# vganapati/CT_PVAE

Measured on AMD Instinct MI355X. Metric: projections/sec (fwd+adj) 128x128 foam, 20 angles; fraction of HBM roofline, higher is better.
Workload: dtype f32; 1 GPU; batch=50/GPU 128x128 foam, 20 angles, P=184, rotate nearest fwd + tf_compat adj; objects_per_gpu=50, n_pixel=128, angles=20, num_proj_pix=184, parallelism=batch-shard x1, forward_plan=u16 taps, launch=19 replays of a HIP graph of 100 steps + 66 steps launched from Python

## Files before the change

ct_pvae_amd/_lib.py:

```python
import ctypes
import os

_HERE = os.path.dirname(os.path.abspath(__file__))
LIB_PATH = os.path.join(_HERE, "libctpvae_radon.so")

NEAREST, BILINEAR = 0, 1
NOISE = {"gaussian": 0, "poisson": 1}
BWD_TF_COMPAT, BWD_EXACT = 0, 1
SIDDON_STORE = {"raysum": 0, "sirt": 1, "tv_dual": 2, "gaussian": 3, "poisson": 4, "ratio": 5}
EINVAL, EHIP, ENODEV = -1, -2, -3
ABI_VERSION = 3400

_c_int, _c_float, _vp = ctypes.c_int, ctypes.c_float, ctypes.c_void_p
_ip = ctypes.POINTER(ctypes.c_int)

SIGNATURES = {
    "ctpvae_abi_version": (_c_int, []),
    "ctpvae_last_error": (ctypes.c_char_p, []),
    "ctpvae_device_count": (_c_int, []),
    "ctpvae_tune_set": (_c_int, [ctypes.c_char_p, _c_int]),
    "ctpvae_tune_active": (_c_int, []),
    "ctpvae_num_proj_pix": (_c_int, [_c_int, _c_int]),
    "ctpvae_pad_amounts": (_c_int, [_c_int, _c_int, _ip, _ip]),
    "ctpvae_rotate_transforms_f32": (_c_int, [_vp, _c_int, _c_int, _c_int, _vp, _vp, _vp]),
    "ctpvae_rotate_transforms_host_f32": (_c_int, [_vp, _c_int, _c_int, _c_int, _vp, _vp]),
    "ctpvae_rotate_fwd_planned_sel_f32": (_c_int, [_vp, _c_int, _c_int, _c_int, _c_int, _c_int, _c_int, _vp, _vp, _c_int, _vp, _vp]),
    "ctpvae_rotate_fwd_planned_loglik_sel_f32": (_c_int, [_vp, _c_int, _c_int, _c_int, _c_int, _c_int, _c_int, _vp, _vp, _c_int,
                                                          _vp, _vp, _c_int, _vp, _c_float, _vp, _vp, _vp, _vp]),
    "ctpvae_rotate_cplan_supported": (_c_int, [_c_int, _c_int, _c_int, _c_int, _c_int, _c_int]),
    "ctpvae_rotate_cplan_bytes": (ctypes.c_longlong, [_c_int, _c_int, _c_int, _c_int, _c_int]),
    "ctpvae_rotate_cplan_build_f32": (_c_int, [_vp, _c_int, _c_int, _c_int, _c_int, _c_int, _c_int, _c_int, _vp, _vp]),
    "ctpvae_rotate_cplan_overflowed": (_c_int, [_vp, _c_int, _c_int, _c_int, _c_int, _c_int, _vp]),
    "ctpvae_rotate_fwd_compact_f32": (_c_int, [_vp, _c_int, _c_int, _c_int, _c_int, _c_int, _c_int, _vp, _vp, _c_int, _c_int, _vp,
                                               _vp, _c_int, _vp, _c_float, _vp, _vp, _vp, _vp, _vp, _vp]),
    "ctpvae_rotate_fwd_compact_noise_f32": (_c_int, [_vp, _c_int, _c_int, _c_int, _c_int, _c_int, _c_int, _vp, _vp, _c_int, _c_int, _vp,
                                                     _vp, _c_int, _vp, _c_float, _c_int, _vp, _vp, _vp, _vp, _vp, _vp]),
    "ctpvae_loglik_tasks_per_row": (_c_int, [_c_int, _c_int]),
    "ctpvae_loglik_part_floats": (ctypes.c_longlong, [_c_int, _c_int, _c_int, _c_int]),
    "ctpvae_loglik_object_sums_f32": (_c_int, [_vp, _c_int, _c_int, _c_int, _c_int, _vp, _vp]),
    "ctpvae_rotate_bwd_sel_scaled_f32": (_c_int, [_vp, _c_int, _c_int, _c_int, _c_int, _vp, _vp, _c_int, _c_int, _c_int, _c_int,
                                                  _c_int, _vp, ctypes.c_longlong, _vp, _vp]),
    "ctpvae_rotate_bwd4_plan_bytes": (ctypes.c_longlong, [_c_int, _c_int, _c_int, _c_int, _c_int]),
    "ctpvae_rotate_bwd4_plan_build_f32": (_c_int, [_vp, _c_int, _c_int, _c_int, _c_int, _c_int, _c_int, _c_int, _vp, _vp]),
    "ctpvae_rotate_bwd_planned_sel_scaled_f32": (_c_int, [_vp, _c_int, _c_int, _c_int, _c_int, _c_int, _c_int, _vp, _vp, _c_int,
                                                          _c_int, _vp, ctypes.c_longlong, _vp, _vp]),
    "ctpvae_rotate_fwd_f32": (_c_int, [_vp, _c_int, _c_int, _c_int, _c_int, _c_int, _c_int, _c_int, _vp, _c_int,
                                       _c_int, _vp, _vp]),
    "ctpvae_rotate_fwd_f64": (_c_int, [_vp, _c_int, _c_int, _c_int, _c_int, _c_int, _c_int, _c_int, _vp, _c_int,
                                       _c_int, _vp, _vp]),
    "ctpvae_rotate_bwd_f64": (_c_int, [_vp, _c_int, _c_int, _c_int, _c_int, _vp, _c_int, _c_int, _c_int, _c_int,
                                       _c_int, _c_int, _vp, _vp]),
    "ctpvae_rotate_tile_shape": (_c_int, [_c_int, _c_int, _c_int, ctypes.POINTER(ctypes.c_int), ctypes.POINTER(ctypes.c_int)]),
    "ctpvae_rotate_fwd_tiled_workspace_bytes": (ctypes.c_longlong, [_c_int, _c_int, _c_int, _c_int, _c_int, _c_int, _c_int]),
    "ctpvae_rotate_fwd_tiled_f32": (_c_int, [_vp, _c_int, _c_int, _c_int, _c_int, _c_int, _c_int, _c_int, _vp, _c_int, _vp,
                                             _vp, _vp]),
    "ctpvae_rotate_fwd_tiled_interp_f32": (_c_int, [_vp, _c_int, _c_int, _c_int, _c_int, _c_int, _c_int, _c_int, _vp, _c_int, _c_int,
                                                    _vp, _vp, _vp]),
    "ctpvae_rotate_fwd_fast_f32": (_c_int, [_vp, _c_int, _c_int, _c_int, _c_int, _c_int, _c_int, _c_int, _vp, _c_int, _vp, _vp]),
    "ctpvae_rotate_fwd_tiled_fast_f32": (_c_int, [_vp, _c_int, _c_int, _c_int, _c_int, _c_int, _c_int, _c_int, _vp, _c_int, _vp,
                                                  _vp, _vp]),
    "ctpvae_rotate_fwd_tiled_loglik_f32": (_c_int, [_vp, _c_int, _c_int, _c_int, _c_int, _c_int, _c_int, _c_int, _vp, _c_int,
                                                    _vp, _vp, _vp, _vp, _c_float, _vp, _vp, _vp, _vp]),
    "ctpvae_rotate_tplan_bytes": (ctypes.c_longlong, [_c_int, _c_int, _c_int, _c_int, _c_int]),
    "ctpvae_rotate_tplan_build_f32": (_c_int, [_vp, _c_int, _c_int, _c_int, _c_int, _c_int, _c_int, _c_int, _vp, _vp]),
    "ctpvae_rotate_tplan_overflowed": (_c_int, [_vp, _c_int, _c_int, _c_int, _c_int, _c_int, _vp]),
    "ctpvae_rotate_fwd_tiled_compact_f32": (_c_int, [_vp, _c_int, _c_int, _c_int, _c_int, _c_int, _c_int, _c_int, _vp, _c_int, _vp,
                                                     _vp, _vp, _vp, _vp, _c_float, _vp, _vp, _vp, _vp, _vp, _vp]),
    "ctpvae_rotate_bwd_f32": (_c_int, [_vp, _c_int, _c_int, _c_int, _c_int, _vp, _c_int, _c_int, _c_int, _c_int,
                                       _c_int, _c_int, _vp, _vp]),
    "ctpvae_rotate_bwd_scaled_f32": (_c_int, [_vp, _c_int, _c_int, _c_int, _c_int, _vp, _c_int, _c_int, _c_int, _c_int,
                                              _c_int, _c_int, _vp, ctypes.c_longlong, _vp, _vp]),
    "ctpvae_rotate_plan_supported": (_c_int, [_c_int, _c_int, _c_int, _c_int, _c_int, _c_int, _c_int]),
    "ctpvae_rotate_plan_bytes": (ctypes.c_longlong, [_c_int, _c_int, _c_int, _c_int, _c_int, _c_int]),
    "ctpvae_rotate_plan_build_f32": (_c_int, [_vp, _vp, _c_int, _c_int, _c_int, _c_int, _c_int, _c_int, _c_int, _vp, _vp,
                                              _vp]),
    "ctpvae_rotate_fwd_planned_f32": (_c_int, [_vp, _c_int, _c_int, _c_int, _c_int, _c_int, _c_int, _vp, _vp, _vp]),
    "ctpvae_rotate_fwd_planned_form": (_c_int, [_c_int, _c_int, _c_int, _c_int, _c_int, _c_int, _c_int]),
    "ctpvae_rotate_fwd_planned_loglik_f32": (_c_int, [_vp, _c_int, _c_int, _c_int, _c_int, _c_int, _c_int, _vp, _vp, _vp, _vp,
                                                      _c_float, _vp, _vp, _vp, _vp]),
    "ctpvae_rotate_bwd_planned_f32": (_c_int, [_vp, _c_int, _c_int, _c_int, _c_int, _c_int, _c_int, _vp, _vp, _vp]),
    "ctpvae_rotate_bwd_planned_scaled_f32": (_c_int, [_vp, _c_int, _c_int, _c_int, _c_int, _c_int, _c_int, _vp, _vp,
                                                      ctypes.c_longlong, _vp, _vp]),
    "ctpvae_rotate_exact_plan_bytes": (ctypes.c_longlong, [_c_int, _c_int, _c_int, _c_int, _c_int]),
    "ctpvae_rotate_exact_plan_build_f32": (_c_int, [_vp, _vp, _c_int, _c_int, _c_int, _c_int, _c_int, _c_int, _c_int, _vp, _vp]),
    "ctpvae_rotate_exact_plan_overflowed": (_c_int, [_vp, _c_int, _c_int, _c_int, _c_int, _c_int, _vp]),
    "ctpvae_rotate_bwd_exact_planned_f32": (_c_int, [_vp, _c_int, _c_int, _c_int, _c_int, _c_int, _c_int, _vp, _vp, _vp]),
    "ctpvae_rotate_exact_wplan_bytes": (ctypes.c_longlong, [_c_int, _c_int, _c_int]),
    "ctpvae_rotate_exact_wplan_build_f32": (_c_int, [_vp, _vp, _c_int, _c_int, _c_int, _c_int, _c_int, _c_int, _c_int, _c_int, _vp, _vp]),
    "ctpvae_rotate_exact_wplan_overflowed": (_c_int, [_vp, _c_int, _c_int, _c_int, _vp]),
    "ctpvae_rotate_bwd_exact_wplan_f32": (_c_int, [_vp, _c_int, _c_int, _c_int, _c_int, _vp, _c_int, _c_int, _c_int, _c_int, _vp,
                                                              _vp, _vp]),
    "ctpvae_rotate_bwd_step_plan_bytes": (ctypes.c_longlong, [_c_int, _c_int, _c_int]),
    "ctpvae_rotate_bwd_step_plan_build_f32": (_c_int, [_vp, _c_int, _c_int, _c_int, _c_int, _c_int, _c_int, _c_int, _vp, _vp]),
    "ctpvae_rotate_bwd_step_plan_overflowed": (_c_int, [_vp, _c_int, _c_int, _c_int, _vp]),
    "ctpvae_rotate_bwd_stepped_scaled_f32": (_c_int, [_vp, _c_int, _c_int, _c_int, _c_int, _vp, _c_int, _c_int, _c_int, _c_int, _vp, _vp,
                                                      ctypes.c_longlong, _vp, _vp]),
    "ctpvae_siddon_dx": (_c_int, [_c_int, _c_int, _c_int]),
    "ctpvae_siddon_tables_f32": (_c_int, [_vp, _c_int, _vp, _vp, _vp]),
    "ctpvae_siddon_fwd_f32": (_c_int, [_vp, _c_int, _c_int, _c_int, _vp, _vp, _vp, _c_int, _c_int, _c_float, _vp,
                                       _vp]),
    "ctpvae_siddon_bwd_workspace_bytes": (ctypes.c_longlong, [_c_int, _c_int, _c_int, _c_int, _c_int]),
    "ctpvae_siddon_bwd_prepare_f32": (_c_int, [_c_int, _c_int, _vp, _vp, _vp, _c_int, _c_int, _c_float, _vp, _vp]),
    "ctpvae_siddon_bwd_prepared_f32": (_c_int, [_vp, _c_int, _c_int, _c_int, _vp, _vp, _vp, _c_int, _c_int, _c_float, _vp, _vp, _vp,
                                                _vp]),
    "ctpvae_siddon_fwd_workspace_bytes": (ctypes.c_longlong, [_c_int, _c_int, _c_int]),
    "ctpvae_siddon_fwd_ws_f32": (_c_int, [_vp, _c_int, _c_int, _c_int, _vp, _vp, _vp, _c_int, _c_int, _c_float, _vp, _vp, _vp, _vp,
                                          _vp]),
    "ctpvae_siddon_fwd_ws_tv_dual_f32": (_c_int, [_vp, _c_int, _c_int, _c_int, _vp, _vp, _vp, _c_int, _c_int, _c_float, _vp, _vp, _vp,
                                                  _vp, _vp]),
    "ctpvae_siddon_bwd_tv_primal_f32": (_c_int, [_vp, _c_int, _c_int, _c_int, _vp, _vp, _vp, _c_int, _c_int, _c_float, _vp, _vp,
                                                 _c_float, _vp, _vp, _vp, _vp, _vp, _vp, _vp, _vp]),
    "ctpvae_siddon_fwd_loglik_f32": (_c_int, [_vp, _c_int, _c_int, _c_int, _vp, _vp, _vp, _c_int, _c_int, _c_float, _vp, _c_int, _vp, _vp,
                                              _c_int, _vp, _c_float, _vp, _vp, _vp, _vp, _vp]),
    "ctpvae_siddon_fwd_loglik_noise_f32": (_c_int, [_vp, _c_int, _c_int, _c_int, _vp, _vp, _vp, _c_int, _c_int, _c_float, _vp, _c_int, _vp,
                                                    _vp, _c_int, _vp, _c_float, _c_int, _vp, _vp, _vp, _vp, _vp]),
    "ctpvae_siddon_bwd_sel_scaled_f32": (_c_int, [_vp, _c_int, _c_int, _c_int, _vp, _vp, _vp, _c_int, _c_int, _c_float, _vp, _c_int, _vp,
                                                  _vp, ctypes.c_longlong, _vp, _vp]),
    "ctpvae_siddon_fwd_ratio_f32": (_c_int, [_vp, _c_int, _c_int, _c_int, _vp, _vp, _vp, _c_int, _c_int, _c_float, _vp, _c_int, _vp, _vp,
                                             _vp, _vp]),
    "ctpvae_siddon_bwd_sel_mul_f32": (_c_int, [_vp, _c_int, _c_int, _c_int, _vp, _vp, _vp, _c_int, _c_int, _c_float, _vp, _c_int, _vp,
                                               _vp, _vp, _vp]),
    "ctpvae_siddon_bwd_sel_pml_f32": (_c_int, [_vp, _c_int, _c_int, _c_int, _vp, _vp, _vp, _c_int, _c_int, _c_float, _vp, _c_int, _vp,
                                               _vp, _c_float, _c_float, _c_int, _vp, _vp, _vp]),
    "ctpvae_siddon_fwd_resid_f32": (_c_int, [_vp, _c_int, _c_int, _c_int, _vp, _vp, _vp, _c_int, _c_int, _c_float, _vp, _vp, _vp,
                                             _vp]),
    "ctpvae_siddon_bwd_f32": (_c_int, [_vp, _c_int, _c_int, _c_int, _vp, _vp, _vp, _c_int, _c_int, _c_float, _vp, _vp, _vp]),
    "ctpvae_siddon_rownorm_f32": (_c_int, [_c_int, _c_int, _vp, _vp, _vp, _c_int, _c_int, _c_float, _vp, _vp]),
    "ctpvae_siddon_fwd_form": (_c_int, [_c_int, _c_int, _c_int, _c_int, _c_int, _c_int]),
    "ctpvae_fbp_filter_f64": (_c_int, [_vp, _c_int, _c_int, _vp, _vp, _vp]),
    "ctpvae_fbp_backproject_f64": (_c_int, [_vp, _c_int, _c_int, _c_int, _vp, _vp, _c_int, _c_int, _vp, _vp]),
    "ctpvae_fbp_backproject_bwd_f64": (_c_int, [_vp, _c_int, _c_int, _c_int, _vp, _vp, _c_int, _c_int, ctypes.c_double,
                                                ctypes.c_double, ctypes.c_double, _vp, _vp]),
    "ctpvae_fbp_backproject_geom_f64": (_c_int, [_vp, _c_int, _c_int, _c_int, _vp, _vp, _c_int, _c_int, ctypes.c_double,
                                                 ctypes.c_double, ctypes.c_double, _vp, _vp]),
    "ctpvae_gridrec_tables_bytes": (ctypes.c_longlong, [_c_int, _c_int]),
    "ctpvae_gridrec_tables_host_f32": (_c_int, [_c_int, _c_int, _c_float, _vp, _c_int, _vp, _vp]),
    "ctpvae_gridrec_workspace_bytes": (ctypes.c_longlong, [_c_int, _c_int, _c_int]),
    "ctpvae_gridrec_f32": (_c_int, [_vp, _c_int, _c_int, _c_int, _vp, _c_int, _c_int, _vp, _vp, _vp]),
    "ctpvae_poisson_loglik_fwd_f32": (_c_int, [_vp, _vp, _vp, _c_int, _c_int, _c_int, _vp, _vp, _vp]),
    "ctpvae_poisson_loglik_bwd_f32": (_c_int, [_vp, _vp, _vp, _vp, _c_int, _c_int, _c_int, _vp, _vp, _vp]),
    "ctpvae_loglik_fwd_f32": (_c_int, [_vp, _vp, _vp, _c_int, _c_int, _c_int, _vp, _c_float, _vp, _vp]),
    "ctpvae_poisson_measure_f32": (_c_int, [_vp, _vp, _c_int, _c_int, _c_int, _c_float, ctypes.c_ulonglong, _vp, _vp]),
    "ctpvae_philox4x32_10": (_c_int, [_vp, _vp, _vp]),
    "ctpvae_loglik_bwd_f32": (_c_int, [_vp, _vp, _vp, _vp, _c_int, _c_int, _c_int, _vp, _c_float, _vp, _vp, _vp]),
    "ctpvae_hmc_state_floats": (_c_int, [_c_int]),
    "ctpvae_hmc_init_f32": (_c_int, [_vp, _c_int, _c_int, _c_int, _vp, _vp, _c_int, _vp, _vp, _c_float, _c_int, _vp, _vp, _vp, _vp,
                                     _c_float, _vp]),
    "ctpvae_hmc_run_f32": (_c_int, [_vp, _c_int, ctypes.c_uint, _c_int, _c_int, _vp, _vp, _c_int, _vp, _vp, _c_float, _c_int, _vp, _vp,
                                    _vp, _c_int, _c_int, ctypes.c_uint, ctypes.c_uint, ctypes.c_ulonglong, _vp, _vp, _vp, _vp, _vp]),
    "ctpvae_tn_head_fwd_f32": (_c_int, [_vp, _vp, _c_int, _c_int, ctypes.c_longlong, ctypes.c_ulonglong, ctypes.c_uint, _vp, _vp, _vp, _vp,
                                        _vp]),
    "ctpvae_tn_head_bwd_f32": (_c_int, [_vp, _vp, _c_int, _c_int, ctypes.c_longlong, ctypes.c_ulonglong, ctypes.c_uint, _vp, _vp, _vp, _vp,
                                        _vp, _vp]),
    "ctpvae_tn_head_uniforms_host_f32": (_c_int, [_c_int, _c_int, ctypes.c_longlong, ctypes.c_ulonglong, ctypes.c_uint, _vp]),
    "ctpvae_beta_head_fwd_f32": (_c_int, [_vp, _vp, _c_int, _c_int, ctypes.c_longlong, ctypes.c_ulonglong, ctypes.c_uint, _c_float, _vp, _vp,
                                          _vp, _vp, _vp]),
    "ctpvae_beta_head_bwd_f32": (_c_int, [_vp, _vp, _c_int, _c_int, ctypes.c_longlong, ctypes.c_ulonglong, ctypes.c_uint, _c_float, _vp, _vp,
                                          _vp, _vp, _vp]),
    "ctpvae_beta_head_words_host_u32": (_c_int, [_c_int, _c_int, ctypes.c_longlong, ctypes.c_ulonglong, ctypes.c_uint, _c_int, _c_int, _vp]),
    "ctpvae_tn_marginals_workspace_bytes": (ctypes.c_longlong, [_c_int, _c_int, ctypes.c_uint]),
    "ctpvae_tn_marginals_f32": (_c_int, [_vp, _vp, _c_int, _c_int, ctypes.c_longlong, ctypes.c_ulonglong, ctypes.c_uint, ctypes.c_uint,
                                         _c_float, _c_float, _c_int, _vp, _vp, _vp, _vp, _vp]),
    "ctpvae_tn_marginals_bin_host_f32": (_c_int, [_vp, ctypes.c_longlong, _c_float, _c_float, _c_int, _vp]),
    "ctpvae_latent_fwd_f32": (_c_int, [_vp, _c_int, _c_int, _c_int, _c_float, ctypes.c_longlong, ctypes.c_ulonglong, ctypes.c_uint,
                                       ctypes.c_uint, _vp, _vp, _vp, _vp, _vp, _vp]),
    "ctpvae_latent_bwd_f32": (_c_int, [_vp, _c_int, _c_int, _c_int, _c_float, ctypes.c_longlong, ctypes.c_ulonglong, ctypes.c_uint,
                                       ctypes.c_uint, _vp, _vp, _vp, _vp, _vp]),
    "ctpvae_latent_draws_host_f32": (_c_int, [_c_int, _c_int, _c_int, ctypes.c_longlong, ctypes.c_ulonglong, ctypes.c_uint, ctypes.c_uint,
                                              _vp]),
    "ctpvae_periodic_pad_fwd_f32": (_c_int, [_vp, _c_int, _c_int, _c_int, _c_int, _c_int, _c_int, _c_int, _vp, _vp]),
    "ctpvae_periodic_pad_bwd_f32": (_c_int, [_vp, _c_int, _c_int, _c_int, _c_int, _c_int, _c_int, _c_int, _vp, _vp]),
    "ctpvae_maxout_fwd_f32": (_c_int, [_vp, _c_int, _c_int, _vp, _vp, _vp]),
    "ctpvae_maxout_bwd_f32": (_c_int, [_vp, _vp, _c_int, _c_int, _vp, _vp]),
    "ctpvae_dropout_fwd_f32": (_c_int, [_vp, _c_int, _c_int, ctypes.c_longlong, ctypes.c_ulonglong, ctypes.c_uint, ctypes.c_uint,
                                        ctypes.c_uint, _c_float, _vp, _vp]),
    "ctpvae_dropout_bwd_f32": (_c_int, [_vp, _c_int, _c_int, ctypes.c_longlong, ctypes.c_ulonglong, ctypes.c_uint, ctypes.c_uint,
                                        ctypes.c_uint, _c_float, _vp, _vp]),
    "ctpvae_dropout_pad_fwd_f32": (_c_int, [_vp, _c_int, _c_int, _c_int, _c_int, _c_int, _c_int, _c_int, _c_int, ctypes.c_longlong,
                                            ctypes.c_ulonglong, ctypes.c_uint, ctypes.c_uint, ctypes.c_uint, _c_float, _vp, _vp]),
    "ctpvae_dropout_pad_bwd_f32": (_c_int, [_vp, _c_int, _c_int, _c_int, _c_int, _c_int, _c_int, _c_int, _c_int, ctypes.c_longlong,
                                            ctypes.c_ulonglong, ctypes.c_uint, ctypes.c_uint, ctypes.c_uint, _c_float, _vp, _vp]),
    "ctpvae_dropout_keep_host_u8": (_c_int, [_c_int, _c_int, ctypes.c_longlong, ctypes.c_ulonglong, ctypes.c_uint, ctypes.c_uint,
                                             ctypes.c_uint, _vp]),
    "ctpvae_merit_tile": (_c_int, []),
    "ctpvae_merit_workspace_bytes": (ctypes.c_longlong, [_c_int, _c_int, _c_int]),
    "ctpvae_merit_f32": (_c_int, [_vp, _vp, _c_int, _c_int, _c_int, _vp, _vp, _vp]),
    "ctpvae_merit_f64": (_c_int, [_vp, _vp, _c_int, _c_int, _c_int, _vp, _vp, _vp]),
}

_lib = None


class RadonLibraryError(RuntimeError):
    """The HIP extension is missing or a HIP call inside it failed."""


def load():
    global _lib
    if _lib is None:
        if not os.path.exists(LIB_PATH):
            raise RadonLibraryError(
                f"{LIB_PATH} is missing: build it with `make -C {os.path.join(_HERE, 'csrc')}` "
                "(or `python -c 'import __graft_entry__ as g; g.build()'`). There is no CPU fallback.")
        lib = ctypes.CDLL(LIB_PATH)
        for name, (res, args) in SIGNATURES.items():
            fn = getattr(lib, name)
            fn.restype = res
            fn.argtypes = args
        if lib.ctpvae_abi_version() != ABI_VERSION:
            raise RadonLibraryError(f"{LIB_PATH} has ABI {lib.ctpvae_abi_version()}, this binding needs {ABI_VERSION}: rebuild it")
        _lib = lib
    return _lib


NODE_NAME = "_ctpvae_torch_node"
NODE_DIR = os.path.join(_HERE, "_torch_node")
NODE_PATH = os.path.join(NODE_DIR, NODE_NAME + ".so")
_node = False


def _node_stamp(src, hdr):
    import hashlib
    import torch
    h = hashlib.sha256()
    for path in (src, hdr):
        with open(path, "rb") as f:
            h.update(f.read())
    return f"abi={ABI_VERSION} src={h.hexdigest()[:32]} torch={torch.__version__}\n"


# ... 97 lines not shown
```

ct_pvae_amd/csrc/common.h:

```cpp
#pragma once
#include <hip/hip_runtime.h>
#include <atomic>
#include <cstdarg>
#include <cstdio>
#include <cstdlib>

#include "../../include/ctpvae_radon.h"

namespace ctpvae {

char *err_buf();
int fail(int code, const char *fmt, ...);

#define CTPVAE_REQUIRE(cond, ...)                                   \
    do {                                                            \
        if (!(cond)) return ::ctpvae::fail(CTPVAE_EINVAL, __VA_ARGS__); \
    } while (0)

#define CTPVAE_HIP(call)                                                                      \
    do {                                                                                      \
        hipError_t e_ = (call);                                                               \
        if (e_ != hipSuccess)                                                                 \
            return ::ctpvae::fail(CTPVAE_EHIP, "%s failed: %s", #call, hipGetErrorString(e_)); \
    } while (0)

#define CTPVAE_LAUNCH_CHECK(name)                                                             \
    do {                                                                                      \
        hipError_t e_ = hipGetLastError();                                                    \
        if (e_ != hipSuccess)                                                                 \
            return ::ctpvae::fail(CTPVAE_EHIP, "launch of %s failed: %s", name, hipGetErrorString(e_)); \
    } while (0)

constexpr int kMaxLdsBytes = 160 * 1024;

struct SliceScale {
    const float *ptr;
    long long stride;
    __device__ __forceinline__ float at(int s) const { return ptr ? ptr[(long long)s * stride] : 1.0f; }
};

enum StorePolicy { kStorePlain = 0, kStoreWriteThrough = 1, kStoreNonTemporal = 2 };
template <int ST> __device__ __forceinline__ void store_f32(float v, float *p)
{
    if constexpr (ST == kStoreWriteThrough) __hip_atomic_store(p, v, __ATOMIC_RELAXED, __HIP_MEMORY_SCOPE_AGENT);
    else if constexpr (ST == kStoreNonTemporal) __builtin_nontemporal_store(v, p);
    else *p = v;
}
template <int ST> __device__ __forceinline__ void store_f32x2(float v0, float v1, float *p)
{
    typedef float f2_t __attribute__((ext_vector_type(2)));
    const f2_t v = {v0, v1};
    if constexpr (ST == kStoreWriteThrough)
        __hip_atomic_store(reinterpret_cast<unsigned long long *>(p), __builtin_bit_cast(unsigned long long, v), __ATOMIC_RELAXED,
                           __HIP_MEMORY_SCOPE_AGENT);
    else if constexpr (ST == kStoreNonTemporal) __builtin_nontemporal_store(v, reinterpret_cast<f2_t *>(p));
    else *reinterpret_cast<f2_t *>(p) = v;
}

#define CTPVAE_SET_MAX_LDS_ONCE(kernel, seen)                                                                     \
    do {                                                                                                          \
        int dev_ = 0;                                                                                             \
        CTPVAE_HIP(hipGetDevice(&dev_));                                                                          \
        const unsigned long long bit_ = 1ull << (dev_ & 63);                                                      \
        if (dev_ >= 64 || !((seen).load(std::memory_order_acquire) & bit_)) {                                     \
            CTPVAE_HIP(hipFuncSetAttribute((const void *)(kernel), hipFuncAttributeMaxDynamicSharedMemorySize,    \
                                           ::ctpvae::kMaxLdsBytes));                                              \
            if (dev_ < 64) (seen).fetch_or(bit_, std::memory_order_release);                                      \
        }                                                                                                         \
    } while (0)

#define CTPVAE_REQUIRE_NO_STATIC_LDS(kernel, name, seen)                                                           \
    do {                                                                                                          \
        int dev_ = 0;                                                                                             \
        CTPVAE_HIP(hipGetDevice(&dev_));                                                                          \
        const unsigned long long bit_ = 1ull << (dev_ & 63);                                                      \
        const int fake_ = ::ctpvae::knob(::ctpvae::kKnobFakeStaticLds);                                            \
        if (dev_ >= 64 || fake_ > 0 || !((seen).load(std::memory_order_acquire) & bit_)) {                        \
            hipFuncAttributes fa_;                                                                                \
            CTPVAE_HIP(hipFuncGetAttributes(&fa_, (const void *)(kernel)));                                       \
            const long long static_ = (long long)fa_.sharedSizeBytes + (fake_ > 0 ? fake_ : 0);                    \
            if (static_ != 0)                                                                                     \
                return ::ctpvae::fail(CTPVAE_EHIP, "%s was built with %lld bytes of static LDS: its gathers address LDS " \
                                      "absolutely and need the dynamic array at address 0 -- rebuild the library (no "    \
                                      "__shared__ variables in these kernels)", name, static_);                   \
            if (dev_ < 64 && fake_ <= 0) (seen).fetch_or(bit_, std::memory_order_release);                        \
        }                                                                                                         \
    } while (0)

enum Knob {
    kKnobNoPlan, kKnobForceGeneric, kKnobNs, kKnobG, kKnobWaves, kKnobBns, kKnobBw, kKnobSegNs, kKnobSegChunk,
    kKnobSegPpt, kKnobTiledNs, kKnobTiledG, kKnobSiddonNs, kKnobSiddonThreads, kKnobSiddonPpb, kKnobMaxSlices,
    kKnobSiddonBwdNs, kKnobSiddonBwdChunks, kKnobNoCompact, kKnobSkew0, kKnobTiledSort, kKnobTiledPair, kKnobAffine, kKnobFakeStaticLds, kKnobFoldSums, kKnobTiledXcd, kKnobTiledWaves, kKnobTiledTh, kKnobReduceWaves, kKnobStepNs, kKnobStepLdsKb, kKnobTiledForce, kKnobBsort, kKnobMixG, kKnobMixG2, kKnobMixU1, kKnobNoMagic, kKnobMixG1, kKnobMixG3, kKnobMixU2, kKnobBrsplit, kKnobFwdFew, kKnobWtStores, kKnobBwdTail, kKnobCount
};
int knob(Knob k);

inline int store_policy(int rule)
{
    const int v = knob(kKnobWtStores);
    return v >= 0 && v <= 2 ? v : rule;
}

inline int max_slices_per_launch()
{
    const int v = knob(kKnobMaxSlices);
    return (v >= 1 && v <= 65535) ? v : 65535;
}

inline int ceil_div(int a, int b) { return (a + b - 1) / b; }

}
```

ct_pvae_amd/csrc/core.hip:

```cpp
#include <cmath>
#include <cstring>

#include "common.h"

namespace ctpvae {

char *err_buf()
{
    static thread_local char buf[512] = {0};
    return buf;
}

int fail(int code, const char *fmt, ...)
{
    va_list ap;
    va_start(ap, fmt);
    vsnprintf(err_buf(), 512, fmt, ap);
    va_end(ap);
    return code;
}

static const char *const kKnobNames[kKnobCount] = {
    "NO_PLAN", "FORCE_GENERIC", "NS", "G", "WAVES", "BNS", "BW", "SEG_NS", "SEG_CHUNK", "SEG_PPT", "TILED_NS", "TILED_G",
    "SIDDON_NS", "SIDDON_THREADS", "SIDDON_PPB", "MAX_SLICES", "SIDDON_BWD_NS", "SIDDON_BWD_CHUNKS", "NO_COMPACT", "SKEW0", "TILED_SORT", "TILED_PAIR", "AFFINE", "FAKE_STATIC_LDS", "FOLD_SUMS", "TILED_XCD", "TILED_WAVES", "TILED_TH", "REDUCE_WAVES", "STEP_NS", "STEP_LDS_KB", "TILED_FORCE", "BSORT", "MIXG", "MIXG_G2", "MIXG_U1", "NO_MAGIC", "MIXG_G1", "MIXG_G3", "MIXG_U2", "BRSPLIT", "FWD_FEW", "WT_STORES", "BWD_TAIL"};
static std::atomic<int> g_knobs[kKnobCount];
static int find_knob(const char *name)
{
    for (int k = 0; k < kKnobCount; ++k)
        if (strcmp(name, kKnobNames[k]) == 0) return k;
    return -1;
}
static const bool g_knobs_loaded = [] {
    for (int k = 0; k < kKnobCount; ++k) {
        int v = -1;
        char env[64];
        if (k == kKnobNoPlan || k == kKnobForceGeneric) {
            snprintf(env, sizeof env, "CTPVAE_%s", kKnobNames[k]);
            if (getenv(env) != nullptr) v = 1;
        } else {
            snprintf(env, sizeof env, "CTPVAE_TUNE_%s", kKnobNames[k]);
            if (const char *e = getenv(env)) v = atoi(e);
        }
        g_knobs[k].store(v, std::memory_order_relaxed);
    }
    return true;
}();
int knob(Knob k) { return g_knobs[k].load(std::memory_order_relaxed); }

__host__ __device__ static void inv3x3(const float m[9], float out[9])
{
    float a[3][6];
#pragma unroll
    for (int r = 0; r < 3; ++r)
#pragma unroll
        for (int c = 0; c < 3; ++c) {
            a[r][c] = m[3 * r + c];
            a[r][3 + c] = (r == c) ? 1.0f : 0.0f;
        }
#pragma unroll
    for (int k = 0; k < 3; ++k) {
        int p = k;
        for (int r = k + 1; r < 3; ++r)
            if (fabsf(a[r][k]) > fabsf(a[p][k])) p = r;
        if (p != k)
            for (int c = 0; c < 6; ++c) {
                float t = a[k][c];
                a[k][c] = a[p][c];
                a[p][c] = t;
            }
        for (int r = k + 1; r < 3; ++r) {
            const float f = a[r][k] / a[k][k];
            for (int c = k; c < 6; ++c) a[r][c] = a[r][c] - f * a[k][c];
        }
    }
    for (int c = 3; c < 6; ++c)
        for (int r = 2; r >= 0; --r) {
            float v = a[r][c];
            for (int q = r + 1; q < 3; ++q) v = v - a[r][q] * a[q][c];
            a[r][c] = v / a[r][r];
        }
    for (int r = 0; r < 3; ++r)
        for (int c = 0; c < 3; ++c) out[3 * r + c] = a[r][3 + c];
}

__host__ __device__ static void transform_rows(float theta, float hm1, float wm1, float *t8, float *tinv8)
{
    const float ang = -theta;
    const float c = (float)cos((double)ang);
    const float s = (float)sin((double)ang);
    const float cw = c * wm1, sh = s * hm1, sw = s * wm1, ch = c * hm1;
    const float xo = (wm1 - (cw - sh)) / 2.0f;
    const float yo = (hm1 - (sw + ch)) / 2.0f;
    const float t[8] = {c, -s, xo, s, c, yo, 0.0f, 0.0f};
    for (int k = 0; k < 8; ++k) t8[k] = t[k];
    if (tinv8) {
        const float m[9] = {t[0], t[1], t[2], t[3], t[4], t[5], t[6], t[7], 1.0f};
        float inv[9];
        inv3x3(m, inv);
        for (int k = 0; k < 8; ++k) tinv8[k] = inv[k] / inv[8];
    }
}

__global__ void rotate_transforms_kernel(const float *__restrict__ theta, int A, float hm1, float wm1,
                                         float *__restrict__ T8, float *__restrict__ Tinv8)
{
    const int a = blockIdx.x * blockDim.x + threadIdx.x;
    if (a >= A) return;
    transform_rows(theta[a], hm1, wm1, T8 + 8 * a, Tinv8 ? Tinv8 + 8 * a : nullptr);
}

}

using namespace ctpvae;

extern "C" {

int ctpvae_abi_version(void) { return CTPVAE_ABI_VERSION; }

int ctpvae_tune_set(const char *name, int value)
{
    CTPVAE_REQUIRE(name != nullptr, "tune_set: null name");
    if (strcmp(name, "*") == 0) {
        for (int k = 0; k < kKnobCount; ++k) g_knobs[k].store(-1, std::memory_order_relaxed);
        return CTPVAE_OK;
    }
    const int k = find_knob(name);
    CTPVAE_REQUIRE(k >= 0, "tune_set: unknown knob '%s'", name);
    g_knobs[k].store(value < 0 ? -1 : value, std::memory_order_relaxed);
    return CTPVAE_OK;
}

int ctpvae_tune_active(void)
{
    int n = 0;
    for (int k = 0; k < kKnobCount; ++k) n += g_knobs[k].load(std::memory_order_relaxed) >= 0;
    return n;
}

const char *ctpvae_last_error(void) { return err_buf(); }

int ctpvae_device_count(void)
{
    int n = 0;
    hipError_t e = hipGetDeviceCount(&n);
    if (e != hipSuccess) return fail(CTPVAE_ENODEV, "hipGetDeviceCount: %s", hipGetErrorString(e));
    return n;
}

int ctpvae_num_proj_pix(int nx, int ny)
{
    CTPVAE_REQUIRE(nx > 0 && ny > 0, "num_proj_pix: sizes must be positive (got %d, %d)", nx, ny);
    const double v = std::sqrt((double)((long long)nx * nx + (long long)ny * ny)) + 2.0;
    return (int)(std::ceil(v / 2.0) * 2.0);
}

int ctpvae_pad_amounts(int n, int P, int *lo, int *hi)
{
    CTPVAE_REQUIRE(lo && hi, "pad_amounts: null output");
    CTPVAE_REQUIRE(n > 0 && P >= n, "pad_amounts: need 0 < n <= P (got n=%d, P=%d)", n, P);
    *lo = (P - n) / 2;
    *hi = *lo + ((P - n) % 2);
    return CTPVAE_OK;
}

int ctpvae_rotate_transforms_host_f32(const float *theta, int A, int H, int W, float *T8, float *Tinv8)
{
    CTPVAE_REQUIRE(theta && T8, "rotate_transforms_host: null pointer");
    CTPVAE_REQUIRE(A > 0 && H > 0 && W > 0, "rotate_transforms_host: bad sizes A=%d H=%d W=%d", A, H, W);
    for (int a = 0; a < A; ++a)
        transform_rows(theta[a], (float)H - 1.0f, (float)W - 1.0f, T8 + 8 * a, Tinv8 ? Tinv8 + 8 * a : nullptr);
    return CTPVAE_OK;
}

int ctpvae_rotate_transforms_f32(const float *theta_dev, int A, int H, int W, float *T8_dev,
                                 float *Tinv8_dev, ctpvae_stream_t stream)
{
    CTPVAE_REQUIRE(theta_dev && T8_dev, "rotate_transforms: null pointer");
// ... 11 lines not shown
```

ct_pvae_amd/csrc/rotate_plan.h:

```cpp
#pragma once
#include <hip/hip_runtime.h>

#include "common.h"

namespace ctpvae {

struct PlanGeom {
    int H, W, PH, PW, py, px, A;
};

__host__ __device__ inline int pitch_mod32_is_1(int w) { return w + ((1 - (w & 31)) & 31); }

__host__ __device__ inline int lane_to_bin(int PW, int jb, int lane)
{
    const int c = PW >> 1;
    return lane < 32 ? c - 32 * (jb + 1) + lane : c + 32 * jb + (lane - 32);
}
__host__ __device__ inline int num_bin_blocks(int PW) { return (PW - (PW >> 1) + 31) / 32; }

typedef const __attribute__((address_space(3))) float *lds_cptr;
typedef __attribute__((address_space(3))) float *lds_ptr;
typedef const __attribute__((address_space(1))) float *glb_cptr;

__device__ __forceinline__ int wave_min_i(int v)
{
#pragma unroll
    for (int off = 32; off > 0; off >>= 1) v = min(v, __shfl_xor(v, off, 64));
    return v;
}
__device__ __forceinline__ int wave_max_i(int v)
{
#pragma unroll
    for (int off = 32; off > 0; off >>= 1) v = max(v, __shfl_xor(v, off, 64));
    return v;
}

typedef float f32x2 __attribute__((ext_vector_type(2)));
template <int NS> struct SliceVec { typedef float type; };
template <> struct SliceVec<2> { typedef f32x2 type; };
constexpr int kMaxSelAngles = 256;
struct SelHost {
    unsigned w[kMaxSelAngles / 2];
    __host__ __device__ void set(int k, int a) { w[k >> 1] = (w[k >> 1] & ~(0xffffu << (16 * (k & 1)))) | ((unsigned)a << (16 * (k & 1))); }
    __device__ __forceinline__ int get(int k) const { return (int)((w[k >> 1] >> (16 * (k & 1))) & 0xffffu); }
};
inline int check_plan_geom(const char *who, int H, int W, int PH, int PW, int py, int px, int A)
{
    CTPVAE_REQUIRE(H > 0 && W > 0 && A > 0, "%s: sizes must be positive (H=%d W=%d A=%d)", who, H, W, A);
    CTPVAE_REQUIRE(py >= 0 && px >= 0 && PH >= H + py && PW >= W + px,
                   "%s: the %dx%d slice at (%d,%d) does not fit the %dx%d canvas", who, H, W, py, px, PH, PW);
    CTPVAE_REQUIRE((long long)PH * PW < (1ll << 24), "%s: canvas too large for fp32 index arithmetic", who);
    return CTPVAE_OK;
}

}
```

ct_pvae_amd/csrc/rotate_plan.hip:

```cpp
#include <algorithm>
#include <atomic>
#include <climits>
#include <cstdlib>
#include <type_traits>

#include "common.h"
#include "lds_stage.h"
#include "loglik_math.h"
#include "rotate_plan.h"
#include "tune_stamps.h"

namespace ctpvae {

struct FwdLayout {
    int nJB, PWpad, NG, Galloc, pitch, zero, skew0;
    long long off_cls, off_clist, off_first, off_rng, off_idx, bytes;
};
constexpr int kBwdPitch = 257;
constexpr int kBwdChunk = 64;
struct BwdLayout {
    int nXB, Wpad, NA16, pitchg, chunkA;
    long long bytes;
};

static FwdLayout fwd_layout(const PlanGeom &g)
{
    FwdLayout L;
    L.nJB = num_bin_blocks(g.PW);
    L.PWpad = L.nJB * 64;
    L.NG = ceil_div(g.PH, 8);
    L.Galloc = L.NG + 8;
    L.skew0 = knob(kKnobSkew0) > 0 ? 1 : 0;
    L.pitch = L.skew0 ? (g.W + 31) / 32 * 32 : pitch_mod32_is_1(g.W);
    if (L.skew0) L.Galloc += 6;
    L.zero = g.H * L.pitch;
    L.off_cls = 0;
    L.off_clist = (long long)g.A * 4;
    L.off_first = (L.off_clist + 2ll * (g.A + 1) * 4 + 8 + 255) / 256 * 256;
    L.off_rng = (L.off_first + (long long)g.A * L.PWpad * 4 + 255) / 256 * 256;
    L.off_idx = (L.off_rng + (long long)g.A * L.nJB * 8 + 255) / 256 * 256;
    L.bytes = L.off_idx + (long long)g.A * L.Galloc * L.PWpad * 16;
    return L;
}
static int bwd_tail_dwords(int A, int dup)
{
    const int r = A % 16;
    return dup == 1 && r >= 1 && r <= 12 ? (r + 3) / 4 : 0;
}
static BwdLayout bwd_layout(const PlanGeom &g, int dup = 1)
{
    BwdLayout L;
    L.nXB = ceil_div(g.W, 64);
    L.Wpad = L.nXB * 64;
    L.NA16 = ceil_div(g.A * dup, 16);
    L.pitchg = kBwdPitch;
    L.chunkA = std::min(L.NA16 * 16, kBwdChunk);
    L.bytes = (long long)L.NA16 * g.H * L.Wpad * 16;
    L.bytes = (L.bytes + 255) / 256 * 256 + (long long)bwd_tail_dwords(g.A, dup) * g.H * L.Wpad * 4;
    return L;
}
static bool fwd_plan_fits(const PlanGeom &g)
{
    const FwdLayout L = fwd_layout(g);
    return L.zero < 65535 && (size_t)(L.zero + 1) * 4 + 16 <= (size_t)kMaxLdsBytes;
}
static bool bwd_plan_fits(const PlanGeom &g) { return g.PW <= 255; }

__device__ __forceinline__ int fwd_tap(const PlanGeom &g, const FwdLayout &L, bool plus, float xj, float yj, float t1,
                                       float t2, float t4, float t5, int i)
{
    const float fi = (float)i;
    const float x = (xj + t1 * fi) + t2;
    const float y = (yj + t4 * fi) + t5;
    const int ix = (int)__builtin_roundf(x) - g.px;
    const int iy = (int)__builtin_roundf(y) - g.py;
    if ((unsigned)ix < (unsigned)g.W && (unsigned)iy < (unsigned)g.H) return iy * L.pitch + (plus ? ix : g.W - 1 - ix);
    return -1;
}
__global__ __launch_bounds__(64) void rotate_fwd_first_kernel(PlanGeom g, const float *__restrict__ T8, FwdLayout L,
                                                              char *__restrict__ plan)
{
    const int a = blockIdx.y, jb = blockIdx.x, lane = threadIdx.x;
    const int j = lane_to_bin(g.PW, jb, lane);
    const float *t = T8 + 8 * a;
    const float t0 = t[0], t1 = t[1], t2 = t[2], t3 = t[3], t4 = t[4], t5 = t[5];
    const bool plus = L.skew0 ? true : (t0 >= 0.0f) == (t3 >= 0.0f);
    int *cls = reinterpret_cast<int *>(plan + L.off_cls);
    int *first = reinterpret_cast<int *>(plan + L.off_first);
    if (jb == 0 && lane == 0) cls[a] = L.skew0 ? (a & 1) : (plus ? 1 : 0);
    const float xj = t0 * (float)j, yj = t3 * (float)j;
    int f = g.PH;
    if ((unsigned)j < (unsigned)g.PW)
        for (int i = 0; i < g.PH; ++i)
            if (fwd_tap(g, L, plus, xj, yj, t1, t2, t4, t5, i) >= 0) {
                f = i;
                break;
            }
    if (L.skew0) {
        int best_steps = INT_MAX, best_start = f;
        for (int sgn = 0; sgn < 2; ++sgn) {
            const float target = sgn ? -1.0f : 1.0f;
            const float alpha = fabsf(t1) < 1e-3f ? 0.0f : (target - t0) / t1;
            const int d = (int)rintf(alpha * (float)(lane & 31));
            int cmin = f < g.PH ? f - d : INT_MAX;
            for (int off = 16; off > 0; off >>= 1) cmin = min(cmin, __shfl_xor(cmin, off, 64));
            const int start = cmin == INT_MAX ? f : d + cmin;
            int last = -1;
            if (f < g.PH)
                for (int i = g.PH - 1; i >= f; --i)
                    if (fwd_tap(g, L, plus, xj, yj, t1, t2, t4, t5, i) >= 0) {
                        last = i;
                        break;
                    }
            int steps = f < g.PH ? last - start + 1 : 0;
            for (int off = 32; off > 0; off >>= 1) steps = max(steps, __shfl_xor(steps, off, 64));
            if (steps < best_steps) {
                best_steps = steps;
                best_start = start;
            }
        }
        f = f < g.PH ? max(best_start, -(1 << 20)) : f;
    }
    first[(size_t)a * L.PWpad + jb * 64 + lane] = f;
}
constexpr int kRngBias = 0x7f7f7f7f;
__global__ __launch_bounds__(64) void rotate_fwd_plan_kernel(PlanGeom g, const float *__restrict__ T8, FwdLayout L,
                                                             char *__restrict__ plan)
{
    const int a = blockIdx.y, jb = blockIdx.x, gq = blockIdx.z, lane = threadIdx.x;
    const int j = lane_to_bin(g.PW, jb, lane);
    const float *t = T8 + 8 * a;
    const float t0 = t[0], t1 = t[1], t2 = t[2], t3 = t[3], t4 = t[4], t5 = t[5];
    const bool plus = L.skew0 ? true : (t0 >= 0.0f) == (t3 >= 0.0f);
    const int *first = reinterpret_cast<const int *>(plan + L.off_first);
    int *rng = reinterpret_cast<int *>(plan + L.off_rng);
    uint4 *idx = reinterpret_cast<uint4 *>(plan + L.off_idx);
    const float xj = t0 * (float)j, yj = t3 * (float)j;
    const int i0 = first[(size_t)a * L.PWpad + jb * 64 + lane] + 8 * gq;
    unsigned e16[8];
    bool any = false;
#pragma unroll
    for (int e = 0; e < 8; ++e) {
        const int i = i0 + e;
        unsigned v = (unsigned)L.zero;
        if (i >= 0 && i < g.PH && (unsigned)j < (unsigned)g.PW) {
            const int tap = fwd_tap(g, L, plus, xj, yj, t1, t2, t4, t5, i);
            if (tap >= 0) {
                v = (unsigned)tap;
                any = true;
            }
        }
        e16[e] = v;
    }
    uint4 q;
    q.x = e16[0] | (e16[1] << 16);
    q.y = e16[2] | (e16[3] << 16);
    q.z = e16[4] | (e16[5] << 16);
    q.w = e16[6] | (e16[7] << 16);
    idx[((size_t)a * L.Galloc + gq) * L.PWpad + jb * 64 + lane] = q;
    if (__any(any) && lane == 0) {
        atomicMin(&rng[(a * L.nJB + jb) * 2 + 0], gq);
        atomicMin(&rng[(a * L.nJB + jb) * 2 + 1], kRngBias - gq);
    }
}

__global__ __launch_bounds__(64) void rotate_bwd_plan_kernel(PlanGeom g, const float *__restrict__ Tinv8, BwdLayout L,
                                                             uint4 *__restrict__ idx, int tail_t)
{
    const int xb = blockIdx.x, yrow = blockIdx.y, a16 = blockIdx.z, lane = threadIdx.x;
    const int xcol = xb * 64 + lane;
    const float fx = (float)(xcol + g.px), fy = (float)(yrow + g.py);
    unsigned w[4] = {0u, 0u, 0u, 0u};
#pragma unroll
    for (int e = 0; e < 16; ++e) {
        const int a = 16 * a16 + e;
        unsigned v = 255u;
        if (a < g.A && xcol < g.W) {
            const float *t = Tinv8 + 8 * a;
            const float x = (t[0] * fx + t[1] * fy) + t[2];
            const float y = (t[3] * fx + t[4] * fy) + t[5];
            const int ix = (int)__builtin_roundf(x), iy = (int)__builtin_roundf(y);
            if ((unsigned)ix < (unsigned)g.PW && (unsigned)iy < (unsigned)g.PH) v = (unsigned)ix;
        }
        w[e >> 2] |= v << (8 * (e & 3));
    }
    idx[((size_t)a16 * g.H + yrow) * L.Wpad + xcol] = make_uint4(w[0], w[1], w[2], w[3]);
    if (tail_t > 0 && a16 == L.NA16 - 1) {
        unsigned *rec = reinterpret_cast<unsigned *>(idx + (size_t)L.NA16 * g.H * L.Wpad) + ((size_t)yrow * L.Wpad + xcol) * tail_t;
#pragma unroll
        for (int d = 0; d < 3; ++d)
            if (d < tail_t) rec[d] = w[d];
    }
}

__global__ __launch_bounds__(64) void rotate_exact_plan_kernel(PlanGeom g, const float *__restrict__ T8,
                                                               const float *__restrict__ Tinv8, BwdLayout L,
                                                               unsigned char *__restrict__ idx, int *__restrict__ overflow)
{
    const int xb = blockIdx.x, yrow = blockIdx.y, a = blockIdx.z, lane = threadIdx.x;
    const int xcol = xb * 64 + lane;
    unsigned hit0 = 255u, hit1 = 255u;
    if (xcol < g.W) {
        const float *ti = Tinv8 + 8 * a, *t = T8 + 8 * a;
        const float fx = (float)(xcol + g.px), fy = (float)(yrow + g.py);
        const int jc = (int)__builtin_roundf((ti[0] * fx + ti[1] * fy) + ti[2]);
        const int ic = (int)__builtin_roundf((ti[3] * fx + ti[4] * fy) + ti[5]);
        int n = 0;
        for (int i = ic - 1; i <= ic + 1; ++i)
            for (int j = jc - 1; j <= jc + 1; ++j) {
                if ((unsigned)i >= (unsigned)g.PH || (unsigned)j >= (unsigned)g.PW) continue;
                const float x = (t[0] * (float)j + t[1] * (float)i) + t[2];
                const float y = (t[3] * (float)j + t[4] * (float)i) + t[5];
                if ((int)__builtin_roundf(x) - g.px == xcol && (int)__builtin_roundf(y) - g.py == yrow) {
                    if (n == 0) hit0 = (unsigned)j;
                    if (n == 1) hit1 = (unsigned)j;
                    ++n;
                }
            }
        if (n > 2) atomicOr(overflow, 1);
    }
    unsigned char *cell = idx + (((size_t)((2 * a) >> 4) * g.H + yrow) * L.Wpad + xcol) * 16 + ((2 * a) & 15);
    cell[0] = (unsigned char)hit0;
    cell[1] = (unsigned char)hit1;
}

__device__ __forceinline__ void unpack2(unsigned pk, int &lo4, int &hi4)
{
    asm("v_lshlrev_b32_sdwa %0, 2, %1 dst_sel:DWORD dst_unused:UNUSED_PAD src0_sel:DWORD src1_sel:WORD_0"
        : "=v"(lo4)
        : "v"(pk));
    asm("v_lshlrev_b32_sdwa %0, 2, %1 dst_sel:DWORD dst_unused:UNUSED_PAD src0_sel:DWORD src1_sel:WORD_1"
        : "=v"(hi4)
        : "v"(pk));
}
__device__ __forceinline__ float lds_at(const float *, int byte_off) { return *(lds_cptr)(size_t)(unsigned)byte_off; }
__device__ __forceinline__ void unpack2x8(unsigned pk, int &lo8, int &hi8)
{
    asm("v_lshlrev_b32_sdwa %0, 3, %1 dst_sel:DWORD dst_unused:UNUSED_PAD src0_sel:DWORD src1_sel:WORD_0"
        : "=v"(lo8)
        : "v"(pk));
    asm("v_lshlrev_b32_sdwa %0, 3, %1 dst_sel:DWORD dst_unused:UNUSED_PAD src0_sel:DWORD src1_sel:WORD_1"
        : "=v"(hi8)
        : "v"(pk));
}
__device__ __forceinline__ void gather8(const float *lds, const uint4 q, f32x2 (&v)[8])
{
    int a[8];
    unpack2x8(q.x, a[0], a[1]);
    unpack2x8(q.y, a[2], a[3]);
    unpack2x8(q.z, a[4], a[5]);
    unpack2x8(q.w, a[6], a[7]);
#pragma unroll
    for (int e = 0; e < 8; ++e) v[e] = *(const __attribute__((address_space(3))) f32x2 *)(size_t)(unsigned)a[e];
}
__device__ __forceinline__ void gather8(const float *lds, const uint4 q, float (&v)[8])
{
    int a0, a1, a2, a3, a4, a5, a6, a7;
    unpack2(q.x, a0, a1);
    unpack2(q.y, a2, a3);
    unpack2(q.z, a4, a5);
    unpack2(q.w, a6, a7);
    v[0] = lds_at(lds, a0);
    v[1] = lds_at(lds, a1);
    v[2] = lds_at(lds, a2);
    v[3] = lds_at(lds, a3);
    v[4] = lds_at(lds, a4);
    v[5] = lds_at(lds, a5);
    v[6] = lds_at(lds, a6);
    v[7] = lds_at(lds, a7);
}

__host__ __device__ inline unsigned div_magic(unsigned d) { return d > 1 ? (unsigned)((1ull << 32) / d) + 1u : 0u; }
__host__ __device__ inline unsigned div_by_magic(unsigned x, unsigned magic) { return magic ? (unsigned)(((unsigned long long)x * magic) >> 32) : x; }
__host__ __device__ inline unsigned div_magic_floor(unsigned d) { return d > 1 ? (unsigned)((1ull << 32) / d) : 0xffffffffu; }
__host__ __device__ inline unsigned div_by_magic_floor(unsigned x, unsigned magic, unsigned d)
{
    const unsigned q = (unsigned)(((unsigned long long)x * magic) >> 32);
    return q + (x - q * d >= d ? 1u : 0u);
}

__global__ __launch_bounds__(64) void rotate_class_list_kernel(int A, FwdLayout L, char *__restrict__ plan)
{
    const int *cls = reinterpret_cast<const int *>(plan + L.off_cls);
    int *clist = reinterpret_cast<int *>(plan + L.off_clist);
    const int lane = threadIdx.x;
    for (int c = 0; c < 2; ++c) {
        int *list = clist + c * (A + 1);
        int n = 0;
        for (int a0 = 0; a0 < A; a0 += 64) {
            const bool in = a0 + lane < A && cls[a0 + lane] == c;
            const unsigned long long m = __ballot(in);
            if (in) list[1 + n + __popcll(m & ((1ull << lane) - 1ull))] = a0 + lane;
            n += __popcll(m);
        }
        if (lane == 0) {
            list[0] = n;
            reinterpret_cast<unsigned *>(clist + 2 * (A + 1))[c] = div_magic((unsigned)n);
        }
    }
}

constexpr int kSelRounds = 4;
#define CTPVAE_PADD(VC) _Pragma("unroll") for (int e = 0; e < 8; ++e) acc += VC[e];
#define CTPVAE_PSTEP(QN, VN, VC, LOADNEXT)    \
                gather8(lds, QN, VN);                                                              \
                LOADNEXT;                                                                          \
                __builtin_amdgcn_sched_barrier(0);                                                 \
                CTPVAE_PADD(VC)
#define CTPVAE_FWD_WALK_U16                                                                        \
            int n = 0;                                                                             \
            for (; n + 4 < ng; n += 4) {    \
                CTPVAE_PSTEP(q1, vb, va, q1 = p[st])                             \
                CTPVAE_PSTEP(q2, va, vb, q2 = p[2 * st])                          \
                CTPVAE_PSTEP(q3, vb, va, q3 = p[3 * st])                          \
                CTPVAE_PSTEP(q0, va, vb, (p += 4 * st, q0 = p[0]))                \
            }                                                                                      \
            if (n + 1 >= ng) {    \
                CTPVAE_PADD(va)                                                                    \
            } else {                                                                               \
                CTPVAE_PSTEP(q1, vb, va, (void)0)                                                  \
                if (n + 2 >= ng) {                                                                 \
                    CTPVAE_PADD(vb)                                                                \
                } else {                                                                           \
                    CTPVAE_PSTEP(q2, va, vb, (void)0)                                              \
                    if (n + 3 >= ng) {                                                             \
                        CTPVAE_PADD(va)                                                            \
                    } else {                                                                       \
                        CTPVAE_PSTEP(q3, vb, va, (void)0)                                          \
                        CTPVAE_PADD(vb)                                                            \
                    }                                                                              \
                }                                                                                  \
            }
template <int NS, bool EPI, bool SEL>
__global__ __launch_bounds__(1024) void rotate_fwd_planned_kernel(const float *__restrict__ img, PlanGeom g, FwdLayout L,
                                                                  const char *__restrict__ plan, int wgs_per_slice,
                                                                  int g_S, float *__restrict__ sino, LogLikEpilogue epi,
                                                                  const int *__restrict__ sel, int n_sel, int affine,
                                                                  int units1, int wgs2, unsigned inv_wgs1, unsigned inv_wgs2, int small_div,
                                                                  int units2, int wgs3, unsigned inv_wgs3)
{
    typedef typename SliceVec<NS>::type vec_t;
    extern __shared__ float lds[];
    const int units = (g_S + NS - 1) / NS;
    auto piece_of = [&](int q, int &u_, int &wg_, int &wgs_) {
        int u0 = 0, nu = units1;
        unsigned inv = inv_wgs1;
        wgs_ = wgs_per_slice;
        const int Q1 = units1 * wgs_per_slice, Q2 = (units2 - units1) * wgs2;
        if (q >= Q1 + Q2) {
            q -= Q1 + Q2;
            u0 = units2;
            nu = units - units2;
            wgs_ = wgs3;
            inv = inv_wgs3;
        } else if (q >= Q1) {
            q -= Q1;
            u0 = units1;
            nu = units2 - units1;
            wgs_ = wgs2;
            inv = inv_wgs2;
        }
        const int octet = small_div ? (int)div_by_magic((unsigned)q >> 3, inv) : q / (8 * wgs_), rem = q - octet * 8 * wgs_;
        if ((octet + 1) * 8 <= nu) {
            wg_ = rem >> 3;
            u_ = u0 + octet * 8 + (rem & 7);
        } else {
            const int ru = small_div ? (int)div_by_magic((unsigned)rem, inv) : rem / wgs_;
            u_ = u0 + octet * 8 + ru;
            wg_ = rem - ru * wgs_;
        }
    };
    int u, wg, wgs = wgs_per_slice;
    [[maybe_unused]] const int q = blockIdx.x;
    if (affine) {
        u = blockIdx.x / wgs_per_slice;
        wg = blockIdx.x - u * wgs_per_slice;
    } else {
        piece_of(q, u, wg, wgs);
    }
    const int s = u * NS;
    const bool has2 = NS == 2 && s + 1 < g_S;
    const int c = wg & 1, gi = wg >> 1, G = wgs >> 1;
    const int lane = threadIdx.x & 63, wave = threadIdx.x >> 6, nwaves = blockDim.x >> 6;
    const float *im = img + (size_t)s * g.H * g.W;
    CTPVAE_PSTAMP(0);

    const int *clist = reinterpret_cast<const int *>(plan + L.off_clist) + c * (g.A + 1);
    const int *rng = reinterpret_cast<const int *>(plan + L.off_rng);
    const uint4 *idx = reinterpret_cast<const uint4 *>(plan + L.off_idx);
    const int A_out = SEL ? n_sel : g.A;
    int sel_a[kSelRounds], sel_rank[kSelRounds], sel_cum[kSelRounds + 1];
    int ncls;
    if constexpr (SEL) {
        const int *cls = reinterpret_cast<const int *>(plan + L.off_cls);
        sel_cum[0] = 0;
#pragma unroll
        for (int r = 0; r < kSelRounds; ++r) {
            const int k = 64 * r + lane;
            int a = 0, cl = -1;
            if (k < n_sel) {
                a = min(max(sel[k], 0), g.A - 1);
                cl = cls[a];
            }
            const unsigned long long m = __ballot(cl == c);
            sel_a[r] = a;
            sel_rank[r] = cl == c ? (int)__popcll(m & ((1ull << lane) - 1ull)) : -1;
            sel_cum[r + 1] = sel_cum[r] + (int)__popcll(m);
        }
        ncls = sel_cum[kSelRounds];
    } else {
        ncls = clist[0];
    }
    [[maybe_unused]] const unsigned inv_ncls = reinterpret_cast<const unsigned *>(plan + L.off_clist + 2ll * (g.A + 1) * 4)[c];
    const int n_gi = affine ? max(0, (ncls - gi + G - 1) / G) : 0;
    const int ntask = affine ? n_gi * L.nJB : ncls * L.nJB;
#ifdef CTPVAE_TUNE_NOIDX
    const size_t st = 0;
#else
    const size_t st = (size_t)L.PWpad;
#endif
    struct Task {
        bool valid;
        int a, k, j, ng;
        const uint4 *p;
        uint4 q0, q1, q2, q3;
        float em[NS], ex[NS];
    };
    [[maybe_unused]] float epnm = 0.0f, einv = 0.0f;
    if constexpr (EPI) epnm = *epi.pnm, einv = 1.0f / epnm;
    auto prepare = [&](int w) -> Task {
        Task t;
        const int m = affine ? w : w * G + gi;
        t.valid = m < ntask;
        t.a = t.k = t.j = t.ng = 0;
        t.p = idx;
        t.q0 = t.q1 = t.q2 = t.q3 = uint4{0, 0, 0, 0};
#pragma unroll
        for (int n = 0; n < NS; ++n) t.em[n] = t.ex[n] = 0.0f;
        if (t.valid) {
            int jb, ai;
            if (affine) {
                jb = m / n_gi;
                ai = gi + G * (m - jb * n_gi);
            } else {
                jb = !SEL && small_div ? (int)div_by_magic((unsigned)m, inv_ncls) : m / ncls;
                ai = m - jb * ncls;
            }
            if constexpr (SEL) {
#pragma unroll
                for (int r = 0; r < kSelRounds; ++r)
                    if (ai >= sel_cum[r] && ai < sel_cum[r + 1]) {
                        const unsigned long long hit = __ballot(sel_rank[r] == ai - sel_cum[r]);
                        const int l = __builtin_amdgcn_readfirstlane((int)__ffsll((long long)hit) - 1);
                        t.a = __builtin_amdgcn_readlane(sel_a[r], l);
                        t.k = 64 * r + l;
                    }
            } else {
                t.k = t.a = clist[1 + ai];
            }
            const int first = rng[(t.a * L.nJB + jb) * 2], last = kRngBias - rng[(t.a * L.nJB + jb) * 2 + 1];
            const int g0 = last >= first ? first : 0;
            t.ng = last >= first ? last - first + 1 : 0;
            t.j = lane_to_bin(g.PW, jb, lane);
            t.p = idx + ((size_t)t.a * L.Galloc + g0) * L.PWpad + jb * 64 + lane;
            t.q0 = t.p[0];
            t.q1 = t.p[st];
            t.q2 = t.p[2 * st];
            t.q3 = t.p[3 * st];
            t.p += 4 * st;
            if constexpr (EPI) {
                const int jc = min(max(t.j, 0), g.PW - 1);
#pragma unroll
                for (int n = 0; n < NS; ++n) {
                    const int sl = min(s + n, g_S - 1);
                    const size_t sa = SEL && epi.dense ? (size_t)sl * g.A + t.a : (size_t)sl * A_out + t.k;
                    t.em[n] = epi.mask[sa];
                    t.ex[n] = epi.meas[sa * g.PW + jc];
                }
            }
        }
        return t;
    };
    Task cur = prepare(wave);
    int *next_task = reinterpret_cast<int *>(lds + (L.zero + 1) * NS);
    if (threadIdx.x == 0) *next_task = nwaves;
// ... 218 lines not shown
#define CTPVAE_BWD_PLANNED_STORE kStoreWriteThrough
#include "rotate_bwd_planned_kernel.h"
#undef CTPVAE_BWD_PLANNED_KERNEL
#undef CTPVAE_BWD_PLANNED_STORE

__global__ __launch_bounds__(64) void rotate_bwd4_plan_kernel(PlanGeom g, const float *__restrict__ Tinv8, int Wpad, int HQ,
                                                              unsigned *__restrict__ idx4)
{
    const int xb = blockIdx.x, yq = blockIdx.y, a = blockIdx.z, lane = threadIdx.x;
    const int xcol = xb * 64 + lane;
    const float *t = Tinv8 + 8 * a;
    const float fx = (float)(xcol + g.px);
    unsigned w = 0u;
#pragma unroll
    for (int e = 0; e < 4; ++e) {
        const int yrow = 4 * yq + e;
        unsigned v = 255u;
        if (yrow < g.H && xcol < g.W) {
            const float fy = (float)(yrow + g.py);
            const float x = (t[0] * fx + t[1] * fy) + t[2];
            const float y = (t[3] * fx + t[4] * fy) + t[5];
            const int ix = (int)__builtin_roundf(x), iy = (int)__builtin_roundf(y);
            if ((unsigned)ix < (unsigned)g.PW && (unsigned)iy < (unsigned)g.PH) v = (unsigned)ix;
        }
        w |= v << (8 * e);
    }
    idx4[((size_t)a * HQ + yq) * Wpad + xcol] = w;
}

template <int NS, bool HOSTSEL, int MAXT = 256>
__global__ __launch_bounds__(MAXT) void rotate_bwd_planned_sel_kernel(const float *__restrict__ gsino, PlanGeom g, int Wpad,
                                                                     int HQ, const unsigned *__restrict__ idx4,
                                                                     const int *__restrict__ sel, int n_sel, int tiles_y,
                                                                     int g_S, SliceScale scale, float *__restrict__ gimg,
                                                                     SelHost selh)
{
    typedef typename SliceVec<NS>::type vec_t;
    constexpr int kChunk = kBwdChunk / NS;
    constexpr int ROW = kBwdPitch * 4 * NS;
    extern __shared__ float lds[];
    const int lane = threadIdx.x & 63, wave = threadIdx.x >> 6, nwaves = blockDim.x >> 6;
    const int nXB = Wpad >> 6, tiles = nXB * tiles_y;
    const int units = (g_S + NS - 1) / NS;
    int u, tile;
    {
        const int per8 = 8 * tiles, octet = blockIdx.x / per8, rem = blockIdx.x - octet * per8;
        if ((octet + 1) * 8 <= units) {
            tile = rem >> 3;
            u = octet * 8 + (rem & 7);
        } else {
            u = octet * 8 + rem / tiles;
            tile = rem - (rem / tiles) * tiles;
        }
    }
    const int s = u * NS;
    const bool has2 = NS == 2 && s + 1 < g_S;
    const float k0 = scale.at(s), k1 = has2 ? scale.at(s + 1) : 1.0f;
    const int xb = tile % nXB, ty = tile / nXB;
    const int xcol = xb * 64 + lane;
    const int yq = min(ty * nwaves + wave, HQ - 1);
    const bool wave_live = ty * nwaves + wave < HQ;
    const float *gs = gsino + (size_t)s * n_sel * g.PW;
    const unsigned *p = idx4 + (size_t)yq * Wpad + xcol;
    const size_t astride = (size_t)HQ * Wpad;
    vec_t acc[4];
#pragma unroll
    for (int e = 0; e < 4; ++e) acc[e] = 0.0f;

    auto load16 = [&](int kbase, unsigned (&q)[16]) {
#pragma unroll
        for (int e = 0; e < 16; ++e) {
            const int k = min(kbase + e, n_sel - 1);
            const int a = min(max(HOSTSEL ? selh.get(k) : sel[k], 0), g.A - 1);
            q[e] = p[(size_t)a * astride];
        }
    };
    for (int kc = 0; kc < n_sel; kc += kChunk) {
        const int nk = min(kChunk, n_sel - kc);
        unsigned q0[16];
        load16(kc, q0);
        if (kc > 0) __syncthreads();
        for (int t = threadIdx.x; t < nk * NS; t += blockDim.x) lds[((t / NS) * kBwdPitch + 255) * NS + (t % NS)] = 0.0f;
        if constexpr (NS == 1) {
            stage_rows(lds, gs + (size_t)kc * g.PW, nk, g.PW, g.PW, kBwdPitch, false, lane, wave, nwaves);
        } else {
            const float *srcs[2] = {gs + (size_t)kc * g.PW, gs + (has2 ? (size_t)n_sel * g.PW : 0) + (size_t)kc * g.PW};
            stage_rows_interleaved<2>(lds, srcs, nk, g.PW, g.PW, kBwdPitch, false, lane, wave, nwaves);
        }
        auto block16 = [&](auto k0_tag) {
            constexpr int K0 = decltype(k0_tag)::value;
            if constexpr (K0 < kChunk) {
                if (K0 >= nk) return;
                unsigned q[16];
                if constexpr (K0 == 0) {
#pragma unroll
                    for (int e = 0; e < 16; ++e) q[e] = q0[e];
                    __syncthreads();
                } else {
                    load16(kc + K0, q);
                }
#pragma unroll
                for (int e = 0; e < 16; ++e) {
                    if (K0 + e < nk) {
                        int b0, b1, b2, b3;
                        unpack4<NS == 1 ? 2 : 3>(q[e], b0, b1, b2, b3);
                        acc[0] += lds_at_vec<NS>(lds, b0 + (K0 + e) * ROW);
                        acc[1] += lds_at_vec<NS>(lds, b1 + (K0 + e) * ROW);
                        acc[2] += lds_at_vec<NS>(lds, b2 + (K0 + e) * ROW);
                        acc[3] += lds_at_vec<NS>(lds, b3 + (K0 + e) * ROW);
                    }
                }
            }
        };
        block16(std::integral_constant<int, 0>{});
        block16(std::integral_constant<int, 16>{});
        block16(std::integral_constant<int, 32>{});
        block16(std::integral_constant<int, 48>{});
    }
    if (xcol < g.W && wave_live) {
#pragma unroll
        for (int e = 0; e < 4; ++e) {
            const int y = 4 * yq + e;
            if (y < g.H) {
                if constexpr (NS == 1) {
                    gimg[((size_t)s * g.H + y) * g.W + xcol] = k0 * acc[e];
                } else {
                    gimg[((size_t)s * g.H + y) * g.W + xcol] = k0 * acc[e].x;
                    if (has2) gimg[((size_t)(s + 1) * g.H + y) * g.W + xcol] = k1 * acc[e].y;
                }
            }
        }
    }
}

}

using namespace ctpvae;

extern "C" {

int ctpvae_rotate_plan_supported(int H, int W, int PH, int PW, int A, int interp, int which)
{
    if (interp != CTPVAE_NEAREST || H <= 0 || W <= 0 || PH < H || PW < W || A <= 0) return 0;
    if (knob(kKnobNoPlan) >= 0) return 0;
    if (which == 0 && knob(kKnobTiledForce) == 1) return 0;
    const PlanGeom g{H, W, PH, PW, 0, 0, A};
    return which == 0 ? (fwd_plan_fits(g) ? 1 : 0) : (bwd_plan_fits(g) ? 1 : 0);
}

long long ctpvae_rotate_plan_bytes(int H, int W, int PH, int PW, int A, int which)
{
    if (H <= 0 || W <= 0 || PH < H || PW < W || A <= 0) return fail(CTPVAE_EINVAL, "rotate_plan_bytes: bad sizes");
    const PlanGeom g{H, W, PH, PW, 0, 0, A};
    return which == 0 ? fwd_layout(g).bytes : bwd_layout(g).bytes;
}

int ctpvae_rotate_plan_build_f32(const float *T8_dev, const float *Tinv8_dev, int A, int H, int W, int PH, int PW, int py,
                                 int px, void *fwd_plan_dev, void *bwd_plan_dev, ctpvae_stream_t stream)
{
    if (int rc = check_plan_geom("rotate_plan_build", H, W, PH, PW, py, px, A)) return rc;
    CTPVAE_REQUIRE(fwd_plan_dev || bwd_plan_dev, "rotate_plan_build: no plan buffer given");
    const PlanGeom g{H, W, PH, PW, py, px, A};
    if (fwd_plan_dev) {
        CTPVAE_REQUIRE(T8_dev, "rotate_plan_build: forward plan needs the forward transforms");
        CTPVAE_REQUIRE(fwd_plan_fits(g), "rotate_plan_build: a %dx%d slice does not fit the forward plan's LDS image", H, W);
        CTPVAE_REQUIRE(A <= 65535, "rotate_plan_build: at most 65535 angles");
        const FwdLayout L = fwd_layout(g);
        CTPVAE_REQUIRE(L.Galloc <= 65535, "rotate_plan_build: canvas too tall");
        CTPVAE_HIP(hipMemsetAsync((char *)fwd_plan_dev + L.off_rng, 0x7f, (size_t)A * L.nJB * 8, (hipStream_t)stream));
        hipLaunchKernelGGL(rotate_fwd_first_kernel, dim3(L.nJB, A), dim3(64), 0, (hipStream_t)stream, g, T8_dev, L,
                           (char *)fwd_plan_dev);
        CTPVAE_LAUNCH_CHECK("rotate_fwd_first_kernel");
        hipLaunchKernelGGL(rotate_fwd_plan_kernel, dim3(L.nJB, A, L.Galloc), dim3(64), 0, (hipStream_t)stream, g, T8_dev, L,
                           (char *)fwd_plan_dev);
        CTPVAE_LAUNCH_CHECK("rotate_fwd_plan_kernel");
        hipLaunchKernelGGL(rotate_class_list_kernel, dim3(1), dim3(64), 0, (hipStream_t)stream, A, L, (char *)fwd_plan_dev);
        CTPVAE_LAUNCH_CHECK("rotate_class_list_kernel");
    }
    if (bwd_plan_dev) {
        CTPVAE_REQUIRE(Tinv8_dev, "rotate_plan_build: backward plan needs the inverted transforms");
        CTPVAE_REQUIRE(bwd_plan_fits(g), "rotate_plan_build: the backward plan stores bins as bytes (PW=%d > 255)", PW);
        CTPVAE_REQUIRE(H <= 65535, "rotate_plan_build: at most 65535 rows");
        const BwdLayout L = bwd_layout(g);
        hipLaunchKernelGGL(rotate_bwd_plan_kernel, dim3(L.nXB, H, L.NA16), dim3(64), 0, (hipStream_t)stream, g, Tinv8_dev, L,
                           (uint4 *)bwd_plan_dev, bwd_tail_dwords(A, 1));
        CTPVAE_LAUNCH_CHECK("rotate_bwd_plan_kernel");
    }
    return CTPVAE_OK;
}

constexpr double kRoundKb = 150.0;
static inline double launch_rounds(long long wgs)
{
    const double real = (double)wgs / 256.0, whole = std::ceil(real);
    return whole > 1.0 ? real + 0.75 * (whole - real) : 1.0;
}

struct FwdShape {
    PlanGeom g;
    FwdLayout L;
    int ns, affine, waves, units, wgs_per_slice, units1, wgs2, units2, wgs3, small_div;
    long long grid;
    size_t shmem;
};
static int fwd_planned_shape(int S, int H, int W, int PH, int PW, int A, bool has_sel, int n_sel, FwdShape &sh)
{
    CTPVAE_REQUIRE(S > 0, "rotate_fwd_planned: need at least one slice");
    if (int rc = check_plan_geom("rotate_fwd_planned", H, W, PH, PW, 0, 0, A)) return rc;
    CTPVAE_REQUIRE(!has_sel || (n_sel >= 1 && n_sel <= 64 * kSelRounds),
                   "rotate_fwd_planned: an angle subset holds 1..%d angles (got %d); build a plan for larger ones",
                   64 * kSelRounds, n_sel);
    const PlanGeom g{H, W, PH, PW, 0, 0, A};
    CTPVAE_REQUIRE(fwd_plan_fits(g), "rotate_fwd_planned: a %dx%d slice does not fit the plan's LDS image", H, W);
    const FwdLayout L = fwd_layout(g);
    const int A_run = has_sel ? n_sel : A;
    const int T = A_run * L.nJB;
    const bool pairs_fit = (size_t)(L.zero + 1) * 8 + 16 <= (size_t)kMaxLdsBytes && S >= 2;
    int ns = 1, G = 1, affine = 0;
    {
        const double task_kb = 0.6 * L.NG;
        const double plan_kb = (double)L.bytes * A_run / A / 1024.0;
        double best = 0.0, best_aff = 0.0;
        int ns_aff = 1, G_aff = 4;
        for (int cand_ns = 1; cand_ns <= (pairs_fit ? 2 : 1); ++cand_ns) {
            const double fill_kb = (double)g.H * g.W * 4.0 * cand_ns / 1024.0;
            const long long cand_units = (S + cand_ns - 1) / cand_ns;
            const double fabric_kb = 1.5 * plan_kb * (double)std::min<long long>(8, cand_units) / 256.0;
            for (int cand = 1; cand <= std::min(12, std::max(1, T / 2)); ++cand) {
                const long long wgs = 2ll * cand_units * cand;
                const double cost = launch_rounds(wgs) * (fill_kb + kRoundKb + task_kb * T / (2.0 * cand)) + fabric_kb;
                if (best == 0.0 || cost <= best * (wgs <= 256 ? 1.03 : 1.0)) {
                    best = best == 0.0 ? cost : std::min(best, cost);
                    ns = cand_ns;
                    G = cand;
                }
            }
            const double fabric_aff = 1.5 * (plan_kb / 8.0 + (double)cand_units * fill_kb * 8.0) / 256.0;
            for (int cand = 4; cand <= 12 && 2 * cand <= std::max(8, T) && cand_units <= 16; cand += 4) {
                const long long wgs = 2ll * cand_units * cand;
                const double cost = (double)((wgs + 255) / 256) * (fill_kb + task_kb * T / (2.0 * cand)) + fabric_aff;
                if (best_aff == 0.0 || cost <= best_aff * 1.03) {
                    best_aff = best_aff == 0.0 ? cost : std::min(best_aff, cost);
                    ns_aff = cand_ns;
                    G_aff = cand;
                }
            }
        }
        const bool can = !has_sel && T >= 8 && best_aff > 0.0;
        if (can && knob(kKnobAffine) != 0 && (knob(kKnobAffine) == 1 || (plan_kb > 3072.0 && best_aff < best))) {
            affine = 1;
            ns = ns_aff;
            G = G_aff;
        }
    }
    if (knob(kKnobNs) >= 0) {
        const int want = knob(kKnobNs) == 2 ? 2 : 1;
        if (want != ns) {
            ns = want;
            affine = 0;
            const double task_kb = 0.6 * L.NG, fill_kb = (double)g.H * g.W * 4.0 * ns / 1024.0;
            const long long cand_units = (S + ns - 1) / ns;
            double best = 0.0;
            for (int cand = 1; cand <= std::min(12, std::max(1, T / 2)); ++cand) {
                const long long wgs = 2ll * cand_units * cand;
                const double cost = launch_rounds(wgs) * (fill_kb + kRoundKb + task_kb * T / (2.0 * cand));
                if (best == 0.0 || cost <= best * (wgs <= 256 ? 1.03 : 1.0)) {
                    best = best == 0.0 ? cost : std::min(best, cost);
                    G = cand;
                }
            }
        }
    }
    const size_t shmem = (size_t)(L.zero + 1) * sizeof(float) * ns + 16;
    const int units = (S + ns - 1) / ns;
    if (knob(kKnobG) > 0) {
        G = knob(kKnobG);
        if (G % 4 != 0) affine = 0;
    }
    const int stage_waves = (int)std::min<size_t>(16, ceil_div((int)(shmem / 1024), 8));
    int waves = std::min(16, std::max(stage_waves, (T + 2 * G - 1) / (2 * G)));
    if (knob(kKnobWaves) > 0) waves = std::min(16, knob(kKnobWaves));
    int wgs_per_slice = 2 * G;
    CTPVAE_REQUIRE((long long)units * wgs_per_slice < (1ll << 31), "rotate_fwd_planned: too many slices");
#ifdef CTPVAE_TUNE_STAMPS
    g_pshape[0] = units, g_pshape[1] = wgs_per_slice, g_pshape[2] = waves, g_pshape[3] = ns, g_pshape[4] = affine;
#endif
    int units1 = units, wgs2 = wgs_per_slice, units2 = units, wgs3 = wgs_per_slice;
    if (!affine && !has_sel && (long long)units * wgs_per_slice > 256 && knob(kKnobMixG) != 0 && knob(kKnobG) <= 0) {
        const double t_fresh = 4.4;
        const int Tc = (T + 1) / 2;
        auto piece_us = [&](int Gx) {
            const int tp = (Tc + Gx - 1) / Gx;
            return t_fresh + std::ceil(tp / 16.0) * (0.072 + 0.0073 * std::min(16, tp)) * L.NG;
        };
        auto launch_us = [&](int G1, int G2, int u1) {
            const long long Q1 = 2ll * u1 * G1, Q2 = 2ll * (units - u1) * G2;
            const double t1 = piece_us(G1), t2 = piece_us(G2);
            const long long r1 = Q1 / 256, rem1 = Q1 % 256;
            double t_free[2] = {r1 * t1, (r1 + 1) * t1};
            long long n_cu[2] = {256 - rem1, rem1}, left = Q2;
            double end = Q1 > 0 ? (rem1 ? t_free[1] : t_free[0]) : 0.0;
            while (left > 0) {
                const int k = n_cu[1] == 0 || t_free[0] <= t_free[1] ? 0 : 1;
                left -= std::min(left, n_cu[k]);
                t_free[k] += t2;
                end = std::max(end, t_free[k]);
            }
            return end;
        };
        int G1 = G, G2 = G, G3 = G;
        struct CutKey { int units, T, NG, G, mix3; };
        struct Cut { CutKey key; int G1, G2, G3, units1, units2; };
        static thread_local Cut cut_cache[8];
        static thread_local unsigned cut_next = 0;
        const CutKey key{units, T, L.NG, G, knob(kKnobMixG3) != 0 ? 1 : 0};
        const Cut *hit = nullptr;
        for (const Cut &c : cut_cache)
            if (c.key.units == key.units && c.key.T == key.T && c.key.NG == key.NG && c.key.G == key.G && c.key.mix3 == key.mix3) hit = &c;
        if (hit) {
            G1 = hit->G1, G2 = hit->G2, G3 = hit->G3, units1 = hit->units1, units2 = hit->units2;
        } else {
        double best = launch_us(G, G, units);
        const int gmax = std::min(12, std::max(1, Tc / 4));
        for (int c1 = 1; c1 <= std::min(8, gmax); ++c1) {
            const int kmax = (int)((2ll * c1 * units) / 256);
            for (int c2 = c1; c2 <= gmax; ++c2)
                for (int k = std::max(0, kmax - 3);; ++k) {
                    const int u1 = std::min(units, (int)((256ll * k) / (2 * c1)));
                    const double t = launch_us(c1, c2, u1);
                    if (t < best * 0.97) best = t, G1 = c1, G2 = c2, units1 = u1;
                    if (u1 == units) break;
                }
        }
        if (units1 == units) G2 = G1;
        G3 = G2;
        if (units1 < units && knob(kKnobMixG3) != 0) {
            auto launch3_us = [&](int c3, int u2) {
                struct Free { double t; long long n; } f[16] = {{0.0, 256}};
                int nf = 1;
                const long long cnt[3] = {2ll * units1 * G1, 2ll * (u2 - units1) * G2, 2ll * (units - u2) * c3};
                const double cost[3] = {piece_us(G1), piece_us(G2), piece_us(c3)};
                double end = 0.0;
                for (int part = 0; part < 3; ++part)
                    for (long long left = cnt[part]; left > 0;) {
                        int k = 0;
                        for (int i = 1; i < nf; ++i) if (f[i].t < f[k].t) k = i;
                        const long long n = std::min(left, f[k].n);
                        if (n < f[k].n && nf < 16) f[nf++] = {f[k].t, f[k].n - n}, f[k].n = n;
                        f[k].t += cost[part];
                        end = std::max(end, f[k].t);
                        left -= n;
                    }
                return end;
            };
            double best3 = launch3_us(G2, units);
            for (int c3 = G2 + 1; c3 <= std::min(gmax, G2 + 3); ++c3)
                for (int u2 = units1 + 4; u2 < units; u2 += 4) {
                    const double t = launch3_us(c3, u2);
                    if (t < best3 * 0.98) best3 = t, G3 = c3, units2 = u2;
                }
            if (G3 == G2) units2 = units;
        }
        cut_cache[cut_next++ % 8] = Cut{key, G1, G2, G3, units1, units2};
        }
        if (knob(kKnobMixG2) > 0 && knob(kKnobMixU1) >= 0)
            G1 = knob(kKnobMixG1) > 0 ? knob(kKnobMixG1) : G, G2 = knob(kKnobMixG2), units1 = std::min(units, knob(kKnobMixU1));
        wgs_per_slice = 2 * G1;
        wgs2 = 2 * G2, wgs3 = 2 * G3;
        if (knob(kKnobMixG2) > 0 && knob(kKnobMixU1) >= 0) wgs3 = wgs2, units2 = units;
        if (knob(kKnobMixG3) > 0 && knob(kKnobMixU2) >= 0)
            wgs3 = 2 * knob(kKnobMixG3), units2 = std::max(units1, std::min(units, knob(kKnobMixU2)));
        waves = std::min(16, std::max(stage_waves, (T + 2 * G1 - 1) / (2 * G1)));
        if (knob(kKnobWaves) > 0) waves = std::min(16, knob(kKnobWaves));
    }
    units2 = std::max(units1, std::min(units2, units));
    const long long grid = (long long)units1 * wgs_per_slice + (long long)(units2 - units1) * wgs2 + (long long)(units - units2) * wgs3;
    CTPVAE_REQUIRE(grid < (1ll << 31), "rotate_fwd_planned: too many slices");
#ifdef CTPVAE_TUNE_STAMPS
    g_pshape[1] = wgs_per_slice, g_pshape[2] = waves, g_pshape[5] = units1, g_pshape[6] = wgs2, g_pshape[7] = units2, g_pshape[8] = wgs3;
#endif
    const int small_div = (grid / 8 + 1) * (long long)std::max(wgs_per_slice, std::max(wgs2, wgs3)) < (1ll << 32) && (long long)A * L.nJB * A < (1ll << 32) &&
                                  knob(kKnobNoMagic) <= 0 ? 1 : 0;
    sh = FwdShape{g, L, ns, affine, waves, units, wgs_per_slice, units1, wgs2, units2, wgs3, small_div, grid, shmem};
    return CTPVAE_OK;
}

constexpr int kFewMaxTasks = 48;
static bool fwd_few_ok(const FwdShape &sh, bool dense, bool img_aligned16)
{
    if (knob(kKnobFwdFew) == 0) return false;
    const int H = sh.g.H, W = sh.g.W;
    const int tasks = ceil_div(sh.g.A * sh.L.nJB, sh.wgs_per_slice);
    if (knob(kKnobFwdFew) != 1 && tasks > kFewMaxTasks) return false;
    return dense && !sh.affine && sh.units1 == sh.units && sh.small_div && !sh.L.skew0 && (W == 64 || W == 128 || W == 256) && H % 4 == 0 &&
           (H / 4) * (W / 64) <= (8 / sh.ns) * sh.waves && img_aligned16;
}

static int launch_fwd_planned(const float *img_dev, int S, int H, int W, int PH, int PW, int A, const void *fwd_plan_dev,
                              float *sino_dev, const LogLikEpilogue &epi, const int *sel_dev, int n_sel,
                              ctpvae_stream_t stream)
{
    CTPVAE_REQUIRE(img_dev && fwd_plan_dev && sino_dev, "rotate_fwd_planned: null pointer");
    FwdShape sh;
    if (int rc = fwd_planned_shape(S, H, W, PH, PW, A, sel_dev != nullptr, n_sel, sh)) return rc;
    const PlanGeom &g = sh.g;
    const FwdLayout &L = sh.L;
    const int ns = sh.ns;
    if (fwd_few_ok(sh, !sel_dev && !epi.lp, (reinterpret_cast<uintptr_t>(img_dev) & 15) == 0)) {
        const char *plan = (const char *)fwd_plan_dev;
        FwdFewArgs k;
        k.clist = reinterpret_cast<const int *>(plan + L.off_clist);
        k.inv_ncls = reinterpret_cast<const unsigned *>(plan + L.off_clist + 2ll * (A + 1) * 4);
        k.rng = reinterpret_cast<const int *>(plan + L.off_rng);
        k.idx = reinterpret_cast<const uint4 *>(plan + L.off_idx);
        k.A = A, k.A1 = A + 1, k.rows = H, k.cs = W == 64 ? 0 : (W == 128 ? 1 : 2), k.src_stride = W, k.pitch = L.pitch, k.zero = L.zero;
        k.PW = PW, k.nJB = L.nJB, k.st = L.PWpad, k.ast = L.Galloc * L.PWpad;
        k.G = sh.wgs_per_slice / 2, k.wgs = sh.wgs_per_slice, k.S = S, k.units = sh.units, k.slice = H * W;
        k.inv_wgs = div_magic((unsigned)sh.wgs_per_slice);
        auto launch_few = [&](auto kernel) -> int {
            static std::atomic<unsigned long long> attr_set{0}, abs_ok{0};
            CTPVAE_REQUIRE_NO_STATIC_LDS(kernel, "rotate_fwd_planned_kernel_few", abs_ok);
            CTPVAE_SET_MAX_LDS_ONCE(kernel, attr_set);
            hipLaunchKernelGGL(kernel, dim3((unsigned)sh.grid), dim3(64 * sh.waves), sh.shmem, (hipStream_t)stream, img_dev, sino_dev, k);
            CTPVAE_LAUNCH_CHECK("rotate_fwd_planned_kernel_few");
            return CTPVAE_OK;
        };
        return ns == 2 ? launch_few(rotate_fwd_planned_kernel_few<2>) : launch_few(rotate_fwd_planned_kernel_few<1>);
    }
    auto launch = [&](auto kernel) -> int {
        static std::atomic<unsigned long long> attr_set{0}, abs_ok{0};
        CTPVAE_REQUIRE_NO_STATIC_LDS(kernel, "rotate_fwd_planned_kernel", abs_ok);
        CTPVAE_SET_MAX_LDS_ONCE(kernel, attr_set);
        hipLaunchKernelGGL(kernel, dim3((unsigned)sh.grid), dim3(64 * sh.waves), sh.shmem, (hipStream_t)stream,
                           img_dev, g, L, (const char *)fwd_plan_dev, sh.wgs_per_slice, S, sino_dev, epi, sel_dev, n_sel, sh.affine, sh.units1, sh.wgs2,
                           div_magic((unsigned)sh.wgs_per_slice), div_magic((unsigned)sh.wgs2), sh.small_div, sh.units2, sh.wgs3, div_magic((unsigned)sh.wgs3));
        CTPVAE_LAUNCH_CHECK("rotate_fwd_planned_kernel");
        return CTPVAE_OK;
    };
    if (sel_dev) {
        if (epi.lp) return ns == 2 ? launch(rotate_fwd_planned_kernel<2, true, true>) : launch(rotate_fwd_planned_kernel<1, true, true>);
        return ns == 2 ? launch(rotate_fwd_planned_kernel<2, false, true>) : launch(rotate_fwd_planned_kernel<1, false, true>);
    }
    if (epi.lp) return ns == 2 ? launch(rotate_fwd_planned_kernel<2, true, false>) : launch(rotate_fwd_planned_kernel<1, true, false>);
    return ns == 2 ? launch(rotate_fwd_planned_kernel<2, false, false>) : launch(rotate_fwd_planned_kernel<1, false, false>);
}

int ctpvae_rotate_fwd_planned_form(int S, int H, int W, int PH, int PW, int A, int img_aligned16)
{
    FwdShape sh;
    if (int rc = fwd_planned_shape(S, H, W, PH, PW, A, false, 0, sh)) return rc;
    return fwd_few_ok(sh, true, img_aligned16 != 0) ? 1 : 0;
}

int ctpvae_rotate_fwd_planned_f32(const float *img_dev, int S, int H, int W, int PH, int PW, int A, const void *fwd_plan_dev,
                                  float *sino_dev, ctpvae_stream_t stream)
{
    return launch_fwd_planned(img_dev, S, H, W, PH, PW, A, fwd_plan_dev, sino_dev, LogLikEpilogue{}, nullptr, 0, stream);
}

int ctpvae_rotate_fwd_planned_sel_f32(const float *img_dev, int S, int H, int W, int PH, int PW, int A,
                                      const void *fwd_plan_dev, const int *angle_idx_dev, int n_idx, float *sino_dev,
                                      ctpvae_stream_t stream)
{
    CTPVAE_REQUIRE(angle_idx_dev, "rotate_fwd_planned_sel: null angle index");
    return launch_fwd_planned(img_dev, S, H, W, PH, PW, A, fwd_plan_dev, sino_dev, LogLikEpilogue{}, angle_idx_dev, n_idx,
                              stream);
}

int ctpvae_rotate_fwd_planned_loglik_f32(const float *img_dev, int S, int H, int W, int PH, int PW, int A,
                                         const void *fwd_plan_dev, const float *mask_dev, const float *meas_dev,
                                         const float *pnm_dev, float eps, float *sino_dev, float *lp_dev,
                                         float *dlp_dev, ctpvae_stream_t stream)
{
    CTPVAE_REQUIRE(mask_dev && meas_dev && pnm_dev && lp_dev, "rotate_fwd_planned_loglik: null pointer");
    return launch_fwd_planned(img_dev, S, H, W, PH, PW, A, fwd_plan_dev, sino_dev,
                              LogLikEpilogue{mask_dev, meas_dev, pnm_dev, eps, lp_dev, dlp_dev, 0}, nullptr, 0, stream);
}

int ctpvae_rotate_fwd_planned_loglik_sel_f32(const float *img_dev, int S, int H, int W, int PH, int PW, int A,
                                             const void *fwd_plan_dev, const int *angle_idx_dev, int n_idx,
                                             const float *mask_dev, const float *meas_dev, int dense_inputs,
                                             const float *pnm_dev, float eps, float *sino_dev, float *lp_dev,
                                             float *dlp_dev, ctpvae_stream_t stream)
{
    CTPVAE_REQUIRE(angle_idx_dev && mask_dev && meas_dev && pnm_dev && lp_dev, "rotate_fwd_planned_loglik_sel: null pointer");
    return launch_fwd_planned(img_dev, S, H, W, PH, PW, A, fwd_plan_dev, sino_dev,
                              LogLikEpilogue{mask_dev, meas_dev, pnm_dev, eps, lp_dev, dlp_dev, dense_inputs ? 1 : 0},
                              angle_idx_dev, n_idx, stream);
}

int ctpvae_rotate_bwd_planned_f32(const float *gsino_dev, int S, int H, int W, int PH, int PW, int A, const void *bwd_plan_dev,
                                  float *gimg_dev, ctpvae_stream_t stream)
{
    return ctpvae_rotate_bwd_planned_scaled_f32(gsino_dev, S, H, W, PH, PW, A, bwd_plan_dev, nullptr, 0, gimg_dev, stream);
}

static int launch_bwd_planned(const float *gsino_dev, int S, int H, int W, int PH, int PW, int A, const void *bwd_plan_dev,
                              const float *scale_dev, long long scale_stride, float *gimg_dev, int dup,
                              ctpvae_stream_t stream)
{
    CTPVAE_REQUIRE(gsino_dev && bwd_plan_dev && gimg_dev, "rotate_bwd_planned: null pointer");
    CTPVAE_REQUIRE(S > 0, "rotate_bwd_planned: need at least one slice");
    if (int rc = check_plan_geom("rotate_bwd_planned", H, W, PH, PW, 0, 0, A)) return rc;
    const PlanGeom g{H, W, PH, PW, 0, 0, A};
    CTPVAE_REQUIRE(bwd_plan_fits(g), "rotate_bwd_planned: the backward plan stores bins as bytes (PW=%d > 255)", PW);
    const BwdLayout L = bwd_layout(g, dup);
    int ns = S >= 2 ? 2 : 1;
    const bool narrow = L.nXB == 1 && H > 32 && (long long)S * ceil_div(H, 16) < 512;
    if (narrow) ns = 1;
    if (knob(kKnobBns) >= 0) ns = (knob(kKnobBns) == 2 && S >= 2) ? 2 : 1;
    const int ppt = ns == 2 ? 2 : 4;
    const int units = ceil_div(S, ns);
    const size_t shmem = (size_t)std::min(ceil_div(L.NA16 * 16, dup), kBwdChunk / ns) * L.pitchg * sizeof(float) * ns;
    const int Aeff = A * dup;
    int waves = 4;
    if (ns == 2) {
        waves = Aeff >= 64 ? (S >= 32 ? 16 : 8) : (S > 16 ? 8 : 4);
        if (Aeff >= 32 && Aeff < 64 && waves == 8 && (long long)units * L.nXB * ceil_div(H, 8 * ppt) > 256 && (long long)units * L.nXB * ceil_div(H, 16 * ppt) <= 256)
            waves = 16;
        if (Aeff >= 64 && S >= 32) {
            auto wgs = [&](int w) { return (long long)units * L.nXB * ceil_div(H, w * ppt); };
            const int w_more = ceil_div(H, ppt * (ceil_div(H, 16 * ppt) + 1));
            if (wgs(8) <= 256)
                waves = 8;
            else if (w_more >= 9 && w_more < 16 && ceil_div((int)wgs(w_more), 256) == ceil_div((int)wgs(16), 256))
                waves = w_more;
        }
    }
    if (dup == 1 && A <= 32 && ns == 2 && S > 16) {
        auto wgs = [&](int w) { return (long long)units * L.nXB * ceil_div(H, w * ppt); };
        const long long r8 = (wgs(8) + 255) / 256, r11 = (wgs(11) + 255) / 256;
        if (r11 < r8 && r11 <= 2 && wgs(11) * 16 >= r11 * 256 * 15) waves = 11;
    }
    if (ns != 2 && Aeff >= 32 && !narrow)
        while (waves < 16 && (long long)units * L.nXB * ceil_div(H, 2 * waves * ppt) >= 200 && waves * ppt < H) waves *= 2;
    while (waves > 1 && (waves / 2) * ppt >= H) waves /= 2;
    if (knob(kKnobBw) > 0) waves = std::min(16, knob(kKnobBw));
    const int rows_per_wg = waves * ppt;
#ifdef CTPVAE_TUNE_STAMPS
    g_pshape[0] = units, g_pshape[1] = L.nXB * ceil_div(H, waves * ppt), g_pshape[2] = waves, g_pshape[3] = ns, g_pshape[4] = 0, g_pshape[5] = units, g_pshape[6] = g_pshape[1];
#endif
    const int tiles_y = ceil_div(H, rows_per_wg);
    const long long nblk = (long long)units * L.nXB * tiles_y;
    CTPVAE_REQUIRE(nblk < (1ll << 31), "rotate_bwd_planned: too many slices");
    const bool small = (nblk / 8) * (long long)(L.nXB * tiles_y) < (1ll << 32) && L.nXB * tiles_y > 1 && knob(kKnobNoMagic) <= 0;
    const bool is_short = dup == 1 && A <= 32;
    const unsigned inv_tiles = is_short ? div_magic_floor((unsigned)(L.nXB * tiles_y)) : (small ? div_magic((unsigned)(L.nXB * tiles_y)) : 0u);
    const unsigned inv_nxb = is_short ? div_magic_floor((unsigned)L.nXB) : div_magic((unsigned)L.nXB);
    const unsigned stage_magic = is_short && PW % 4 == 0 && (reinterpret_cast<uintptr_t>(gsino_dev) & 15) == 0 ? contig_rows_magic(PW) : 0u;
    CTPVAE_REQUIRE(!is_short || H <= 65535, "rotate_bwd_planned: at most 65535 rows (as rotate_plan_build)");
    const int tail_t = is_short && knob(kKnobBwdTail) != 0 ? bwd_tail_dwords(A, dup) : 0;
    const unsigned idx_req = !is_short ? 0u : (tail_t ? kIdxReqTail1 << (tail_t - 1) : kIdxReqTailWhole) | (tail_t == 0 || A > 16 ? kIdxReqFirst : 0u);
    auto launch = [&](auto kernel) -> int {
        static std::atomic<unsigned long long> attr_set{0}, abs_ok{0};
        CTPVAE_REQUIRE_NO_STATIC_LDS(kernel, "rotate_bwd_planned_kernel", abs_ok);
        CTPVAE_SET_MAX_LDS_ONCE(kernel, attr_set);
        hipLaunchKernelGGL(kernel, dim3((unsigned)nblk), dim3(64 * waves), shmem, (hipStream_t)stream, gsino_dev, g, L,
                           (const uint4 *)bwd_plan_dev, tiles_y, S, SliceScale{scale_dev, scale_stride}, gimg_dev,
                           inv_tiles, inv_nxb, stage_magic, idx_req);
        return CTPVAE_OK;
    };
    const int st = is_short ? store_policy(kStoreWriteThrough) : kStorePlain;
    int rc;
    if (dup == 2) {
        if (ns == 2)
            rc = waves <= 4 ? launch(rotate_bwd_planned_kernel<2, 256, 2, 2>) : launch(rotate_bwd_planned_kernel<2, 1024, 2, 2>);
        else
            rc = waves <= 4 ? launch(rotate_bwd_planned_kernel<4, 256, 1, 2>) : launch(rotate_bwd_planned_kernel<4, 1024, 1, 2>);
    } else if (is_short && st == kStoreWriteThrough) {
        if (ns == 2)
            rc = waves <= 4 ? launch(rotate_bwd_planned_kernel_wt<2, 256, 2, 1, true>) : launch(rotate_bwd_planned_kernel_wt<2, 1024, 2, 1, true>);
        else
            rc = waves <= 4 ? launch(rotate_bwd_planned_kernel_wt<4, 256, 1, 1, true>) : launch(rotate_bwd_planned_kernel_wt<4, 1024, 1, 1, true>);
    } else if (is_short) {
        if (ns == 2)
            rc = waves <= 4 ? launch(rotate_bwd_planned_kernel<2, 256, 2, 1, true>) : launch(rotate_bwd_planned_kernel<2, 1024, 2, 1, true>);
        else
            rc = waves <= 4 ? launch(rotate_bwd_planned_kernel<4, 256, 1, 1, true>) : launch(rotate_bwd_planned_kernel<4, 1024, 1, 1, true>);
    } else if (ns == 2) {
        rc = waves <= 4 ? launch(rotate_bwd_planned_kernel<2, 256, 2>) : launch(rotate_bwd_planned_kernel<2, 1024, 2>);
    } else {
        rc = waves <= 4 ? launch(rotate_bwd_planned_kernel<4, 256, 1>) : launch(rotate_bwd_planned_kernel<4, 1024, 1>);
    }
    if (rc) return rc;
    CTPVAE_LAUNCH_CHECK("rotate_bwd_planned_kernel");
    return CTPVAE_OK;
}

int ctpvae_rotate_bwd_planned_scaled_f32(const float *gsino_dev, int S, int H, int W, int PH, int PW, int A,
                                         const void *bwd_plan_dev, const float *scale_dev, long long scale_stride,
                                         float *gimg_dev, ctpvae_stream_t stream)
{
    return launch_bwd_planned(gsino_dev, S, H, W, PH, PW, A, bwd_plan_dev, scale_dev, scale_stride, gimg_dev, 1, stream);
}

long long ctpvae_rotate_bwd4_plan_bytes(int H, int W, int PH, int PW, int A)
{
    if (H <= 0 || W <= 0 || PH < H || PW < W || A <= 0) return fail(CTPVAE_EINVAL, "rotate_bwd4_plan_bytes: bad sizes");
    const PlanGeom g{H, W, PH, PW, 0, 0, A};
    if (!bwd_plan_fits(g) || knob(kKnobNoPlan) >= 0) return 0;
    return (long long)A * ceil_div(H, 4) * (ceil_div(W, 64) * 64) * 4;
}

int ctpvae_rotate_bwd4_plan_build_f32(const float *Tinv8_dev, int A, int H, int W, int PH, int PW, int py, int px,
// ... 111 lines not shown
```

ct_pvae_amd/forward_functions.py:

```python
import math
import os

import ctypes
import weakref

import numpy as np
import torch

from . import _lib

__all__ = ["pad_phantom", "project_tf_fast", "project_tf_low_mem", "num_proj_pix", "pad_amounts", "RotatePlan",
           "rotate_tables", "as_angle_index"]

_current_device = getattr(torch._C, "_cuda_getDevice", torch.cuda.current_device)
_INTERP = {"nearest": _lib.NEAREST, "bilinear": _lib.BILINEAR}
_BACKWARD = {"tf_compat": _lib.BWD_TF_COMPAT, "exact": _lib.BWD_EXACT}
_PRECISION = ("exact", "fast")


def _check_precision(precision, interp):
    if precision not in _PRECISION:
        raise ValueError(f"precision must be one of {list(_PRECISION)} (got {precision!r})")
    if precision == "fast" and interp != "bilinear":
        raise ValueError(f"precision='fast' needs interp='bilinear' (got interp={interp!r}): nearest has no weights to blend")
# ... 140 lines not shown
        self.A = self.T8.shape[0]
        self._lib = _lib.load()
        self._fwd_plan = self._bwd_plan = self._exact_plan = self._bwd4_plan = None
        self._want_bwd_plan = False
        self._want_bwd4 = bool(use_plan and self.interp == _lib.NEAREST and self.mode == _lib.BWD_TF_COMPAT)
        self._want_exact_plan = bool(use_plan and self.mode == _lib.BWD_EXACT and self.interp == _lib.NEAREST)
        self._use_tiles = bool(use_plan)
        self._tile_ws = None
        self._compact = False
        self._part_ws = {}
        self._u16_plan = None
        self._auto_dense_u16 = False
        if use_plan:
            geo = (self.H, self.W, self.PH, self.PW, self.A, self.interp)
            want_compact = plan_format == "compact" or (plan_format == "auto" and self.A >= self.COMPACT_MIN_ANGLES)
            if want_compact and self._lib.ctpvae_rotate_cplan_supported(*geo):
                self._fwd_plan = self._build_compact_plan()
                self._compact = self._fwd_plan is not None
            if self._fwd_plan is None and self._lib.ctpvae_rotate_plan_supported(*geo, 0):
                self._fwd_plan = self._build_plan(0)
            self._auto_dense_u16 = bool(plan_format == "auto" and self._compact and self._lib.ctpvae_rotate_plan_supported(*geo, 0))
            if self._auto_dense_u16:
                self._u16_plan = self._build_plan(0)
            self._want_bwd_plan = bool(self.mode == _lib.BWD_TF_COMPAT and
                                       self._lib.ctpvae_rotate_plan_supported(*geo, 1))
        self._tplan = None
        if (use_plan and self._fwd_plan is None and self.interp == _lib.NEAREST and plan_format != "u16"
                and self.py > 0 and self.px > 0):
            self._tplan = self._build_tile_plan()
        self._step_plan = None
        if (use_plan and self.interp == _lib.NEAREST and self.mode == _lib.BWD_TF_COMPAT and self.py > 0 and self.px > 0
                and self.A <= 65535 and self.H * self.W >= 128 * 128):
            self._step_plan = self._build_step_plan()
        self._exact_bilin_plan = None
        self._subsets = {}
        if use_plan and self.mode == _lib.BWD_EXACT:
            self._build_exact_plans()

    def _build_exact_plans(self):
        if self.interp == _lib.NEAREST:
            self._build_exact_plan()
        if self.H <= 65535 and (self.interp == _lib.BILINEAR or self._exact_plan is None):
            self._build_exact_bilinear_plan()

    def _build_plan(self, which):
        nbytes = self._lib.ctpvae_rotate_plan_bytes(self.H, self.W, self.PH, self.PW, self.A, which)
        _lib.check(nbytes, "rotate_plan_bytes")
        buf = torch.empty(int(nbytes), dtype=torch.uint8, device=self.device)
        with torch.cuda.device(self.device):
            _lib.check(self._lib.ctpvae_rotate_plan_build_f32(
                self.T8.data_ptr(), self.Tinv8.data_ptr(), self.A, self.H, self.W, self.PH, self.PW, self.py, self.px,
                buf.data_ptr() if which == 0 else None, buf.data_ptr() if which == 1 else None, _stream_ptr()),
                "rotate_plan_build")
        return buf

    def _build_compact_plan(self):
        nbytes = self._lib.ctpvae_rotate_cplan_bytes(self.H, self.W, self.PH, self.PW, self.A)
        _lib.check(nbytes, "rotate_cplan_bytes")
        buf = torch.empty(int(nbytes), dtype=torch.uint8, device=self.device)
        with torch.cuda.device(self.device):
            _lib.check(self._lib.ctpvae_rotate_cplan_build_f32(self.T8.data_ptr(), self.A, self.H, self.W, self.PH, self.PW,
                                                               self.py, self.px, buf.data_ptr(), _stream_ptr()),
                       "rotate_cplan_build")
            over = self._lib.ctpvae_rotate_cplan_overflowed(buf.data_ptr(), self.H, self.W, self.PH, self.PW, self.A,
                                                            _stream_ptr())
        _lib.check(over, "rotate_cplan_overflowed")
        return buf if over == 0 else None

    def _build_tile_plan(self):
        nbytes = self._lib.ctpvae_rotate_tplan_bytes(self.H, self.W, self.PH, self.PW, self.A)
        _lib.check(nbytes, "rotate_tplan_bytes")
        if nbytes == 0:
            return None
        buf = torch.empty(int(nbytes), dtype=torch.uint8, device=self.device)
        with torch.cuda.device(self.device):
            _lib.check(self._lib.ctpvae_rotate_tplan_build_f32(self.T8.data_ptr(), self.A, self.H, self.W, self.PH, self.PW, self.py,
                                                               self.px, buf.data_ptr(), _stream_ptr()), "rotate_tplan_build")
            over = self._lib.ctpvae_rotate_tplan_overflowed(buf.data_ptr(), self.H, self.W, self.PH, self.PW, self.A, _stream_ptr())
        _lib.check(over, "rotate_tplan_overflowed")
        return buf if over == 0 else None

    def _get_bwd4_plan(self):
        if self._bwd4_plan is None and self._want_bwd4:
            self._want_bwd4 = False
            nbytes = self._lib.ctpvae_rotate_bwd4_plan_bytes(self.H, self.W, self.PH, self.PW, self.A)
            _lib.check(nbytes, "rotate_bwd4_plan_bytes")
            if nbytes > 0:
                buf = torch.empty(int(nbytes), dtype=torch.uint8, device=self.device)
                with torch.cuda.device(self.device):
                    _lib.check(self._lib.ctpvae_rotate_bwd4_plan_build_f32(self.Tinv8.data_ptr(), self.A, self.H, self.W, self.PH,
                                                                           self.PW, self.py, self.px, buf.data_ptr(),
                                                                           _stream_ptr()), "rotate_bwd4_plan_build")
                self._bwd4_plan = buf
        return self._bwd4_plan

    def _build_exact_plan(self):
        self._want_exact_plan = False
        nbytes = self._lib.ctpvae_rotate_exact_plan_bytes(self.H, self.W, self.PH, self.PW, self.A)
        _lib.check(nbytes, "rotate_exact_plan_bytes")
        if nbytes == 0:
            return
        buf = torch.empty(int(nbytes), dtype=torch.uint8, device=self.device)
        with torch.cuda.device(self.device):
            _lib.check(self._lib.ctpvae_rotate_exact_plan_build_f32(self.T8.data_ptr(), self.Tinv8.data_ptr(), self.A, self.H,
                                                                    self.W, self.PH, self.PW, self.py, self.px, buf.data_ptr(),
                                                                    _stream_ptr()), "rotate_exact_plan_build")
            over = self._lib.ctpvae_rotate_exact_plan_overflowed(buf.data_ptr(), self.H, self.W, self.PH, self.PW, self.A,
                                                                 _stream_ptr())
        _lib.check(over, "rotate_exact_plan_overflowed")
        if over == 0:
            self._exact_plan = buf

    def _build_exact_bilinear_plan(self):
        nbytes = self._lib.ctpvae_rotate_exact_wplan_bytes(self.H, self.W, self.A)
        _lib.check(nbytes, "rotate_exact_wplan_bytes")
        buf = torch.empty(int(nbytes), dtype=torch.uint8, device=self.device)
        with torch.cuda.device(self.device):
            _lib.check(self._lib.ctpvae_rotate_exact_wplan_build_f32(
                self.T8.data_ptr(), self.Tinv8.data_ptr(), self.A, self.H, self.W, self.PH, self.PW, self.py, self.px,
                self.interp, buf.data_ptr(), _stream_ptr()), "rotate_exact_wplan_build")
            over = self._lib.ctpvae_rotate_exact_wplan_overflowed(buf.data_ptr(), self.H, self.W, self.A, _stream_ptr())
        _lib.check(over, "rotate_exact_wplan_overflowed")
        if over == 0:
            self._exact_bilin_plan = buf

    @property
    def planned(self):
        return self._fwd_plan is not None, self._want_bwd_plan

    @property
    def compact(self):
        return self._compact

    def dense_plan(self, S):
        if self._auto_dense_u16 and not (self.COMPACT_DENSE_WINDOW[0] <= S <= self.COMPACT_DENSE_WINDOW[1]):
            if self._u16_plan is None:
                self._u16_plan = self._build_plan(0)
            return self._u16_plan, False
        return self._fwd_plan, self._compact

    def forward_kernel_name(self, S):
        if self.fast:
            return "rotate_fwd_bilin_kernel<FAST>"
        if self._fwd_plan is None:
            return "rotate_fwd_fast_kernel"
        return "rotate_fwd_compact_kernel" if self.dense_plan(S)[1] else "rotate_fwd_planned_kernel"

    def forward_form(self, S, img=None):
        if self.forward_kernel_name(S) != "rotate_fwd_planned_kernel":
            return 0
        aligned = 1 if img is None or img.data_ptr() % 16 == 0 else 0
        return _lib.check(self._lib.ctpvae_rotate_fwd_planned_form(S, self.H, self.W, self.PH, self.PW, self.A, aligned),
                          "rotate_fwd_planned_form")

    def _run_compact(self, img_ptr, S, out_ptr, angles_i=None, n=0, mask=None, meas=None, dense=0, pnm=None, eps=0.0,
                     lp_ptr=None, dlp_ptr=None, part_ptr=None, sum_ptr=None, noise=0):
        if noise:
            return self._lib.ctpvae_rotate_fwd_compact_noise_f32(
                img_ptr, S, self.H, self.W, self.PH, self.PW, self.A, self._fwd_plan.data_ptr(),
                angles_i.data_ptr() if angles_i is not None else None, n,
                1 if (angles_i is not None and angles_i.device.type == "cpu") else 0, mask.data_ptr() if mask is not None else None,
                meas.data_ptr() if meas is not None else None, dense, pnm.data_ptr() if pnm is not None else None,
                ctypes.c_float(eps), noise, out_ptr, lp_ptr, dlp_ptr, part_ptr, sum_ptr, _stream_ptr(self._dev_index))
        return self._lib.ctpvae_rotate_fwd_compact_f32(
            img_ptr, S, self.H, self.W, self.PH, self.PW, self.A, self._fwd_plan.data_ptr(),
            angles_i.data_ptr() if angles_i is not None else None, n,
            1 if (angles_i is not None and angles_i.device.type == "cpu") else 0, mask.data_ptr() if mask is not None else None,
            meas.data_ptr() if meas is not None else None, dense, pnm.data_ptr() if pnm is not None else None,
            ctypes.c_float(eps), out_ptr, lp_ptr, dlp_ptr, part_ptr, sum_ptr, _stream_ptr(self._dev_index))

    def poisson_fused(self, n_sel=None):
        return self._compact and self.interp == _lib.NEAREST and (n_sel is None or 1 <= n_sel <= self.MAX_SEL)

    def _noise_code(self, noise, angles_i):
        if noise not in _lib.NOISE:
            raise ValueError(f"noise must be 'gaussian' or 'poisson' (got {noise!r})")
        code = _lib.NOISE[noise]
        if code and not self.poisson_fused(None if angles_i is None else angles_i.numel()):
            raise ValueError("noise='poisson' is fused into the step-coded (compact) plan's launch only (see poisson_fused): project, "
                             "then call poisson_log_prob on this geometry")
        return code

    def forward_loglik_sums(self, img, mask, meas, pnm, eps, angles_i=None, dense_inputs=False, with_dlp=True, noise="gaussian"):
        if self.interp != _lib.NEAREST:
            raise ValueError("forward_loglik needs a planned or tiled forward (nearest)")
        noise = self._noise_code(noise, angles_i)
        if angles_i is not None and not self.sel_supported(angles_i.numel()):
            if dense_inputs:
                idx = self._sel_dev(angles_i).long()
                mask, meas = mask.index_select(1, idx).contiguous(), meas.index_select(1, idx).contiguous()
            return self.subset(angles_i).forward_loglik_sums(img, mask, meas, pnm, eps, with_dlp=with_dlp)
        with torch.cuda.device(self._dev_index):
            S = img.shape[0]
            sums = _new_output((S,), torch.float32, self._tdev)
            ws = self._tile_workspace(S) if angles_i is None else None
            if ws is not None:
                self._check(img, (self.H, self.W), "img")
                self._check(meas, (self.A, self.PW), "meas")
                self._check(mask, (self.A,), "mask")
                if meas.shape[0] != S or mask.shape[0] != S or pnm.numel() != 1 or pnm.dtype != torch.float32 or pnm.device != img.device:
                    raise ValueError("mask [S][A], meas [S][A][PW] and a one-element float32 pnm on the same device are needed")
                dlp = _new_output((S, self.A, self.PW), torch.float32, self._tdev) if with_dlp else None
                part = self._part_workspace(S, self.A, 1)
                rc = self._lib.ctpvae_rotate_fwd_tiled_compact_f32(
                    img.data_ptr(), S, self.H, self.W, self.PH, self.PW, self.py, self.px, self.T8.data_ptr(), self.A,
                    self._tplan.data_ptr() if self._tplan is not None else None, ws.data_ptr(), mask.data_ptr(), meas.data_ptr(),
                    pnm.data_ptr(), ctypes.c_float(eps), None, None, dlp.data_ptr() if dlp is not None else None,
                    part.data_ptr(), sums.data_ptr(), _stream_ptr(self._dev_index))
                if rc:
                    _lib.check(rc, "rotate_fwd_tiled_compact")
                return sums, dlp
            if not self._compact:
                res = self._forward_loglik(img, mask, meas, pnm, eps, with_dlp=with_dlp, angles_i=angles_i,
                                           dense_inputs=dense_inputs)
                lp = res[1]
                partition = 0 if self._fwd_plan is not None else 1
                _lib.check(self._lib.ctpvae_loglik_object_sums_f32(lp.data_ptr(), S, lp.shape[1], self.PW, partition,
                                                                   sums.data_ptr(), _stream_ptr(self._dev_index)),
                           "loglik_object_sums")
                return sums, (res[2] if with_dlp else None)
            self._check(img, (self.H, self.W), "img")
            n = self.A if angles_i is None else self._check_sel(angles_i)
            n_in = self.A if (angles_i is None or dense_inputs) else n
            self._check(meas, (n_in, self.PW), "meas")
            self._check(mask, (n_in,), "mask")
            if meas.shape[0] != S or mask.shape[0] != S or pnm.numel() != 1 or pnm.dtype != torch.float32 or pnm.device != img.device:
                raise ValueError("mask [S][A], meas [S][A][PW] and a one-element float32 pnm on the same device are needed")
            dlp = _new_output((S, n, self.PW), torch.float32, self._tdev) if with_dlp else None
            part = self._part_workspace(S, n, 0)
            rc = self._run_compact(img.data_ptr(), S, None, angles_i, n if angles_i is not None else 0, mask, meas,
                                   1 if dense_inputs else 0, pnm, eps, None, dlp.data_ptr() if dlp is not None else None,
                                   part.data_ptr(), sums.data_ptr(), noise=noise)
            if rc:
                _lib.check(rc, "rotate_fwd_compact")
            return sums, dlp

    def _part_workspace(self, S, n, partition):
        ws = self._part_ws.get((S, n, partition))
        if ws is None:
            if torch.cuda.is_current_stream_capturing():
                raise RuntimeError("the first per-object-sum call of a shape allocates and zeroes its workspace: run it once before "
                                   "capturing a HIP graph (the zero fill must not be captured: the counters are zeroed ONCE)")
            nfl = self._lib.ctpvae_loglik_part_floats(S, n, self.PW, partition)
            _lib.check(nfl, "loglik_part_floats")
            if len(self._part_ws) >= 8:
                self._part_ws.clear()
            ws = self._part_ws[(S, n, partition)] = torch.zeros((int(nfl),), dtype=torch.float32, device=self._tdev)
        return ws

    def _sel_dev(self, angles_i):
        return angles_i if angles_i.device == self._tdev else angles_i.to(self._tdev)

    SUBSET_CACHE_MAX = 4

    def subset(self, angles_i):
        key = self._subset_key(angles_i) if self.mode == _lib.BWD_EXACT else None
        hit = self._subsets.get(key) if key is not None else None
        if hit is not None and (hit[0] is None or hit[0]() is angles_i):
            return hit[1]
        idx = as_angle_index(angles_i, self._tdev).long()
        use_plan = False if self._fwd_plan is not None else self._use_tiles
        sub = RotatePlan(None, self.H, self.W, self._pad, self.device, interp=self._interp_name, backward=self._backward_name,
                         use_plan=use_plan, _tables=(self.T8.index_select(0, idx), self.Tinv8.index_select(0, idx)),
                         precision=self.precision)
        if key is not None:
            if not use_plan:
                sub._build_exact_plans()
            if len(self._subsets) >= self.SUBSET_CACHE_MAX:
                self._subsets.pop(next(iter(self._subsets)))
            dev_ref = weakref.ref(angles_i) if key[0] == "dev" else None
            self._subsets[key] = (dev_ref, sub)
        return sub

    @staticmethod
    def _subset_key(angles_i):
        if isinstance(angles_i, torch.Tensor) and angles_i.device.type != "cpu":
            return ("dev", id(angles_i), angles_i._version, angles_i.data_ptr(), tuple(angles_i.shape), angles_i.dtype)
        host = as_angle_index(angles_i, None, keep_host=True)
        return ("host", host.numpy().tobytes())

    def sel_supported(self, n, forward=True):
        if forward:
            return self._fwd_plan is not None and 1 <= n <= self.MAX_SEL
        return self.supports_scale and n >= 1

    def forward(self, img, out=None, angles_i=None):
        n = self.A if angles_i is None else angles_i.numel()
        if img.dim() == 3 and img.shape[0] == 0 and tuple(img.shape[1:]) == (self.H, self.W):
            return out if out is not None else img.new_empty((0, n, self.PW))
        if angles_i is not None and not self.sel_supported(n):
            return self.subset(angles_i).forward(img, out)
        if _current_device() == self._dev_index:
            return self._forward(img, out, angles_i)
        with torch.cuda.device(self._dev_index):
            return self._forward(img, out, angles_i)

    def forward_f64(self, img):
        if self.fast:
            raise ValueError("precision='fast' projects float32 slices only: the float64 path is correctness-first and has no fast form")
        if (img.dim() != 3 or tuple(img.shape[1:]) != (self.H, self.W) or img.dtype is not torch.float64 or not img.is_contiguous()
                or img.device != self._tdev):
            raise ValueError(f"img must be a contiguous float64 tensor [S][{self.H}][{self.W}] on {self._tdev} "
                             f"(got {tuple(img.shape)}, {img.dtype}, {img.device})")
        S = img.shape[0]
        out = _new_output((S, self.A, self.PW), torch.float64, img.device)
        if S == 0:
# ... 606 lines not shown
```

include/ctpvae_radon.h:

```cpp
#ifndef CTPVAE_RADON_H
#define CTPVAE_RADON_H

#ifdef __cplusplus
extern "C" {
#endif

#define CTPVAE_OK 0
#define CTPVAE_EINVAL (-1)
#define CTPVAE_EHIP (-2)
#define CTPVAE_ENODEV (-3)

#define CTPVAE_NOISE_GAUSSIAN 0
#define CTPVAE_NOISE_POISSON 1
#define CTPVAE_NEAREST 0
#define CTPVAE_BILINEAR 1

#define CTPVAE_BWD_TF_COMPAT 0
#define CTPVAE_BWD_EXACT 1

typedef void *ctpvae_stream_t;

#define CTPVAE_ABI_VERSION 3400
int ctpvae_abi_version(void);
const char *ctpvae_last_error(void);
int ctpvae_device_count(void);
int ctpvae_tune_set(const char *name, int value);
int ctpvae_tune_active(void);

int ctpvae_num_proj_pix(int nx, int ny);
int ctpvae_pad_amounts(int n, int P, int *lo, int *hi);

int ctpvae_rotate_transforms_f32(const float *theta_dev, int A, int H, int W, float *T8_dev,
                                 float *Tinv8_dev, ctpvae_stream_t stream);
int ctpvae_rotate_transforms_host_f32(const float *theta, int A, int H, int W, float *T8, float *Tinv8);

int ctpvae_rotate_fwd_f32(const float *img_dev, int S, int H, int W, int PH, int PW, int py, int px,
                          const float *T8_dev, int A, int interp, float *sino_dev,
                          ctpvae_stream_t stream);

int ctpvae_rotate_fwd_f64(const double *img_dev, int S, int H, int W, int PH, int PW, int py, int px,
                          const float *T8_dev, int A, int interp, double *sino_dev, ctpvae_stream_t stream);
int ctpvae_rotate_bwd_f64(const double *gsino_dev, int S, int A, int PH, int PW, const float *T8_dev, int interp, int mode,
                          int H, int W, int py, int px, double *gimg_dev, ctpvae_stream_t stream);

int ctpvae_rotate_tile_shape(int H, int W, int interp, int *tile_h, int *tile_w);
long long ctpvae_rotate_fwd_tiled_workspace_bytes(int S, int H, int W, int PH, int PW, int A, int interp);
int ctpvae_rotate_fwd_tiled_f32(const float *img_dev, int S, int H, int W, int PH, int PW, int py, int px,
                                const float *T8_dev, int A, void *workspace_dev, float *sino_dev,
                                ctpvae_stream_t stream);

int ctpvae_rotate_fwd_tiled_interp_f32(const float *img_dev, int S, int H, int W, int PH, int PW, int py, int px,
                                       const float *T8_dev, int A, int interp, void *workspace_dev, float *sino_dev,
                                       ctpvae_stream_t stream);

int ctpvae_rotate_fwd_fast_f32(const float *img_dev, int S, int H, int W, int PH, int PW, int py, int px,
                               const float *T8_dev, int A, float *sino_dev, ctpvae_stream_t stream);
int ctpvae_rotate_fwd_tiled_fast_f32(const float *img_dev, int S, int H, int W, int PH, int PW, int py, int px,
                                     const float *T8_dev, int A, void *workspace_dev, float *sino_dev,
                                     ctpvae_stream_t stream);

int ctpvae_rotate_fwd_tiled_loglik_f32(const float *img_dev, int S, int H, int W, int PH, int PW, int py, int px,
                                       const float *T8_dev, int A, void *workspace_dev, const float *mask_dev,
                                       const float *meas_dev, const float *pnm_dev, float eps, float *sino_dev,
                                       float *lp_dev, float *dlp_dev, ctpvae_stream_t stream);

long long ctpvae_rotate_tplan_bytes(int H, int W, int PH, int PW, int A);
int ctpvae_rotate_tplan_build_f32(const float *T8_dev, int A, int H, int W, int PH, int PW, int py, int px, void *tplan_dev,
                                  ctpvae_stream_t stream);
int ctpvae_rotate_tplan_overflowed(const void *tplan_dev, int H, int W, int PH, int PW, int A, ctpvae_stream_t stream);
int ctpvae_rotate_fwd_tiled_compact_f32(const float *img_dev, int S, int H, int W, int PH, int PW, int py, int px,
                                        const float *T8_dev, int A, const void *tplan_dev, void *workspace_dev,
                                        const float *mask_dev, const float *meas_dev, const float *pnm_dev, float eps,
                                        float *sino_dev, float *lp_dev, float *dlp_dev, float *lp_part_dev, float *lp_sum_dev,
                                        ctpvae_stream_t stream);

int ctpvae_rotate_bwd_f32(const float *gsino_dev, int S, int A, int PH, int PW, const float *T8_dev,
                          int interp, int mode, int H, int W, int py, int px, float *gimg_dev,
                          ctpvae_stream_t stream);
int ctpvae_rotate_bwd_scaled_f32(const float *gsino_dev, int S, int A, int PH, int PW, const float *T8_dev,
                                 int interp, int mode, int H, int W, int py, int px, const float *scale_dev,
                                 long long scale_stride, float *gimg_dev, ctpvae_stream_t stream);

int ctpvae_rotate_plan_supported(int H, int W, int PH, int PW, int A, int interp, int which);
long long ctpvae_rotate_plan_bytes(int H, int W, int PH, int PW, int A, int which);
int ctpvae_rotate_plan_build_f32(const float *T8_dev, const float *Tinv8_dev, int A, int H, int W, int PH, int PW,
                                 int py, int px, void *fwd_plan_dev, void *bwd_plan_dev, ctpvae_stream_t stream);
int ctpvae_rotate_fwd_planned_f32(const float *img_dev, int S, int H, int W, int PH, int PW, int A,
                                  const void *fwd_plan_dev, float *sino_dev, ctpvae_stream_t stream);
int ctpvae_rotate_fwd_planned_form(int S, int H, int W, int PH, int PW, int A, int img_aligned16);
int ctpvae_rotate_fwd_planned_loglik_f32(const float *img_dev, int S, int H, int W, int PH, int PW, int A,
                                         const void *fwd_plan_dev, const float *mask_dev, const float *meas_dev,
                                         const float *pnm_dev, float eps, float *sino_dev, float *lp_dev,
                                         float *dlp_dev, ctpvae_stream_t stream);
int ctpvae_rotate_fwd_planned_sel_f32(const float *img_dev, int S, int H, int W, int PH, int PW, int A,
                                      const void *fwd_plan_dev, const int *angle_idx_dev, int n_idx, float *sino_dev,
                                      ctpvae_stream_t stream);
int ctpvae_rotate_fwd_planned_loglik_sel_f32(const float *img_dev, int S, int H, int W, int PH, int PW, int A,
                                             const void *fwd_plan_dev, const int *angle_idx_dev, int n_idx,
                                             const float *mask_dev, const float *meas_dev, int dense_inputs,
                                             const float *pnm_dev, float eps, float *sino_dev, float *lp_dev,
                                             float *dlp_dev, ctpvae_stream_t stream);
int ctpvae_rotate_cplan_supported(int H, int W, int PH, int PW, int A, int interp);
long long ctpvae_rotate_cplan_bytes(int H, int W, int PH, int PW, int A);
int ctpvae_rotate_cplan_build_f32(const float *T8_dev, int A, int H, int W, int PH, int PW, int py, int px, void *cplan_dev,
                                  ctpvae_stream_t stream);
int ctpvae_rotate_cplan_overflowed(const void *cplan_dev, int H, int W, int PH, int PW, int A, ctpvae_stream_t stream);
int ctpvae_rotate_fwd_compact_f32(const float *img_dev, int S, int H, int W, int PH, int PW, int A, const void *cplan_dev,
                                  const int *angle_idx, int n_idx, int idx_on_host, const float *mask_dev,
                                  const float *meas_dev, int dense_inputs, const float *pnm_dev, float eps, float *sino_dev,
                                  float *lp_dev, float *dlp_dev, float *lp_part_dev, float *lp_sum_dev, ctpvae_stream_t stream);
int ctpvae_rotate_fwd_compact_noise_f32(const float *img_dev, int S, int H, int W, int PH, int PW, int A, const void *cplan_dev,
                                        const int *angle_idx, int n_idx, int idx_on_host, const float *mask_dev,
                                        const float *meas_dev, int dense_inputs, const float *pnm_dev, float eps, int noise,
                                        float *sino_dev, float *lp_dev, float *dlp_dev, float *lp_part_dev, float *lp_sum_dev,
                                        ctpvae_stream_t stream);

int ctpvae_rotate_bwd_sel_scaled_f32(const float *gsino_dev, int S, int A_plan, int PH, int PW, const float *Tinv8_dev,
                                     const int *angle_idx_dev, int n_idx, int H, int W, int py, int px,
                                     const float *scale_dev, long long scale_stride, float *gimg_dev,
                                     ctpvae_stream_t stream);

long long ctpvae_rotate_bwd4_plan_bytes(int H, int W, int PH, int PW, int A);
int ctpvae_rotate_bwd4_plan_build_f32(const float *Tinv8_dev, int A, int H, int W, int PH, int PW, int py, int px,
                                      void *plan_dev, ctpvae_stream_t stream);
int ctpvae_rotate_bwd_planned_sel_scaled_f32(const float *gsino_dev, int S, int H, int W, int PH, int PW, int A,
                                             const void *bwd4_plan_dev, const int *angle_idx, int n_idx, int idx_on_host,
                                             const float *scale_dev, long long scale_stride, float *gimg_dev,
                                             ctpvae_stream_t stream);

long long ctpvae_rotate_bwd_step_plan_bytes(int H, int W, int A);
int ctpvae_rotate_bwd_step_plan_build_f32(const float *Tinv8_dev, int A, int H, int W, int PH, int PW, int py, int px, void *plan_dev,
                                          ctpvae_stream_t stream);
int ctpvae_rotate_bwd_step_plan_overflowed(const void *plan_dev, int H, int W, int A, ctpvae_stream_t stream);
int ctpvae_rotate_bwd_stepped_scaled_f32(const float *gsino_dev, int S, int A, int PH, int PW, const float *Tinv8_dev, int H, int W,
                                         int py, int px, const void *step_plan_dev, const float *scale_dev, long long scale_stride,
                                         float *gimg_dev, ctpvae_stream_t stream);

int ctpvae_rotate_bwd_planned_f32(const float *gsino_dev, int S, int H, int W, int PH, int PW, int A,
                                  const void *bwd_plan_dev, float *gimg_dev, ctpvae_stream_t stream);
int ctpvae_rotate_bwd_planned_scaled_f32(const float *gsino_dev, int S, int H, int W, int PH, int PW, int A,
                                         const void *bwd_plan_dev, const float *scale_dev, long long scale_stride,
                                         float *gimg_dev, ctpvae_stream_t stream);

long long ctpvae_rotate_exact_plan_bytes(int H, int W, int PH, int PW, int A);
int ctpvae_rotate_exact_plan_build_f32(const float *T8_dev, const float *Tinv8_dev, int A, int H, int W, int PH, int PW,
                                       int py, int px, void *plan_dev, ctpvae_stream_t stream);
int ctpvae_rotate_exact_plan_overflowed(const void *plan_dev, int H, int W, int PH, int PW, int A, ctpvae_stream_t stream);
int ctpvae_rotate_bwd_exact_planned_f32(const float *gsino_dev, int S, int H, int W, int PH, int PW, int A,
                                        const void *exact_plan_dev, float *gimg_dev, ctpvae_stream_t stream);

long long ctpvae_rotate_exact_wplan_bytes(int H, int W, int A);
int ctpvae_rotate_exact_wplan_build_f32(const float *T8_dev, const float *Tinv8_dev, int A, int H, int W, int PH, int PW,
                                        int py, int px, int interp, void *plan_dev, ctpvae_stream_t stream);
int ctpvae_rotate_exact_wplan_overflowed(const void *plan_dev, int H, int W, int A, ctpvae_stream_t stream);
int ctpvae_rotate_bwd_exact_wplan_f32(const float *gsino_dev, int S, int A, int PH, int PW, const float *Tinv8_dev,
                                      int H, int W, int py, int px, const void *plan_dev, float *gimg_dev,
                                      ctpvae_stream_t stream);

int ctpvae_siddon_dx(int ox, int oz, int pad);
int ctpvae_siddon_tables_f32(const float *theta, int dt, float *sin_out, float *cos_out, int *quadrant_out);
int ctpvae_siddon_fwd_f32(const float *obj_dev, int oy, int ox, int oz, const float *sin_dev,
                          const float *cos_dev, const int *quad_dev, int dt, int dx, float center,
                          float *data_dev, ctpvae_stream_t stream);

long long ctpvae_siddon_bwd_workspace_bytes(int oy, int ox, int oz, int dt, int dx);
int ctpvae_siddon_bwd_prepare_f32(int ox, int oz, const float *sin_dev, const float *cos_dev, const int *quad_dev, int dt, int dx,
                                  float center, void *workspace_dev, ctpvae_stream_t stream);
int ctpvae_siddon_bwd_prepared_f32(const float *data_dev, int oy, int ox, int oz, const float *sin_dev, const float *cos_dev,
                                   const int *quad_dev, int dt, int dx, float center, const void *workspace_dev,
                                   const float *colsum_dev, float *recon_dev, ctpvae_stream_t stream);
int ctpvae_siddon_bwd_f32(const float *data_dev, int oy, int ox, int oz, const float *sin_dev, const float *cos_dev,
                          const int *quad_dev, int dt, int dx, float center, void *workspace_dev, float *recon_dev,
                          ctpvae_stream_t stream);
int ctpvae_siddon_fwd_resid_f32(const float *obj_dev, int oy, int ox, int oz, const float *sin_dev, const float *cos_dev,
                                const int *quad_dev, int dt, int dx, float center, const float *meas_dev,
                                const float *rn2_dev, float *upd_dev, ctpvae_stream_t stream);
long long ctpvae_siddon_fwd_workspace_bytes(int oy, int ox, int oz);
int ctpvae_siddon_fwd_ws_f32(const float *obj_dev, int oy, int ox, int oz, const float *sin_dev, const float *cos_dev,
                             const int *quad_dev, int dt, int dx, float center, const float *meas_dev, const float *rn2_dev,
                             void *workspace_dev, float *data_dev, ctpvae_stream_t stream);
int ctpvae_siddon_rownorm_f32(int ox, int oz, const float *sin_dev, const float *cos_dev, const int *quad_dev, int dt,
                              int dx, float center, float *rn2_dev, ctpvae_stream_t stream);
#define CTPVAE_SIDDON_STORE_RAYSUM 0
#define CTPVAE_SIDDON_STORE_SIRT 1
#define CTPVAE_SIDDON_STORE_TV_DUAL 2
#define CTPVAE_SIDDON_STORE_GAUSSIAN 3
#define CTPVAE_SIDDON_STORE_POISSON 4
#define CTPVAE_SIDDON_STORE_RATIO 5
int ctpvae_siddon_fwd_form(int oy, int ox, int oz, int dt, int dx, int store);
int ctpvae_siddon_fwd_loglik_f32(const float *obj_dev, int oy, int ox, int oz, const float *sin_dev, const float *cos_dev,
                                 const int *quad_dev, int dt_all, int dx, float center, const int *sel_dev, int n_sel,
                                 const float *mask_dev, const float *meas_dev, int dense, const float *pnm_dev, float eps,
                                 void *workspace_dev, float *sino_dev, float *lp_dev, float *dlp_dev, ctpvae_stream_t stream);
int ctpvae_siddon_fwd_loglik_noise_f32(const float *obj_dev, int oy, int ox, int oz, const float *sin_dev, const float *cos_dev,
                                       const int *quad_dev, int dt_all, int dx, float center, const int *sel_dev, int n_sel,
                                       const float *mask_dev, const float *meas_dev, int dense, const float *pnm_dev, float eps,
                                       int noise, void *workspace_dev, float *sino_dev, float *lp_dev, float *dlp_dev,
                                       ctpvae_stream_t stream);
int ctpvae_siddon_bwd_sel_scaled_f32(const float *data_dev, int oy, int ox, int oz, const float *sin_dev, const float *cos_dev,
                                     const int *quad_dev, int dt_all, int dx, float center, const int *sel_dev, int n_sel,
                                     const void *workspace_dev, const float *scale_dev, long long scale_stride, float *recon_dev,
                                     ctpvae_stream_t stream);
int ctpvae_siddon_fwd_ratio_f32(const float *obj_dev, int oy, int ox, int oz, const float *sin_dev, const float *cos_dev,
                                const int *quad_dev, int dt_all, int dx, float center, const int *sel_dev, int n_sel,
                                const float *meas_dev, void *workspace_dev, float *ratio_dev, ctpvae_stream_t stream);
int ctpvae_siddon_bwd_sel_mul_f32(const float *ratio_dev, int oy, int ox, int oz, const float *sin_dev, const float *cos_dev,
                                  const int *quad_dev, int dt_all, int dx, float center, const int *sel_dev, int n_sel,
                                  const void *workspace_dev, const float *colsum_dev, float *x_dev, ctpvae_stream_t stream);
int ctpvae_siddon_bwd_sel_pml_f32(const float *ratio_dev, int oy, int ox, int oz, const float *sin_dev, const float *cos_dev,
                                  const int *quad_dev, int dt_all, int dx, float center, const int *sel_dev, int n_sel,
                                  const void *workspace_dev, const float *colsum_dev, float beta, float delta, int hybrid,
                                  const float *x_in_dev, float *x_out_dev, ctpvae_stream_t stream);
int ctpvae_siddon_fwd_ws_tv_dual_f32(const float *xbar_dev, int oy, int ox, int oz, const float *sin_dev, const float *cos_dev,
                                     const int *quad_dev, int dt, int dx, float center, const float *meas_dev,
                                     const float *sigma_dev, void *workspace_dev, float *p_dev, ctpvae_stream_t stream);
int ctpvae_siddon_bwd_tv_primal_f32(const float *p_dev, int oy, int ox, int oz, const float *sin_dev, const float *cos_dev,
                                    const int *quad_dev, int dt, int dx, float center, const void *workspace_dev,
                                    const float *tau_dev, float lam, float *x_dev, const float *xbar_in_dev, float *xbar_out_dev,
                                    const float *qx_in_dev, const float *qy_in_dev, float *qx_out_dev, float *qy_out_dev,
                                    ctpvae_stream_t stream);

int ctpvae_fbp_filter_f64(const double *sino_dev, int R, int P, const double *hker_dev, double *out_dev,
                          ctpvae_stream_t stream);
int ctpvae_fbp_backproject_f64(const double *filt_dev, int B, int A, int P, const double *cos_dev,
                               const double *sin_dev, int X, int Y, double *recon_dev,
                               ctpvae_stream_t stream);
int ctpvae_fbp_backproject_geom_f64(const double *filt_dev, int B, int A, int P, const double *cos_dev,
                                    const double *sin_dev, int X, int Y, double x0, double y0, double t0,
                                    double *recon_dev, ctpvae_stream_t stream);

int ctpvae_fbp_backproject_bwd_f64(const double *grecon_dev, int B, int A, int P, const double *cos_dev,
                                   const double *sin_dev, int X, int Y, double x0, double y0, double t0,
                                   double *gfilt_dev, ctpvae_stream_t stream);

long long ctpvae_gridrec_tables_bytes(int dt, int dx);
int ctpvae_gridrec_tables_host_f32(int dt, int dx, float center, const float *theta, int filter_name, const float *filter_par,
                                   void *tables);
long long ctpvae_gridrec_workspace_bytes(int dy, int dt, int dx);
int ctpvae_gridrec_f32(const float *data_dev, int dy, int dt, int dx, const void *tables_dev, int ngridx, int ngridy,
                       void *workspace_dev, float *recon_dev, ctpvae_stream_t stream);

int ctpvae_loglik_tasks_per_row(int PW, int partition);
// ... 98 lines not shown
```

Baseline: 109.3 million projections/s.

## Add cost-balanced task dealing for the few-slice forward projection kernel

Adds a plan-build kernel that sorts the forward projection tasks (angle × column-block pieces) by length and partitions them across workgroups with a cost model (binary search on a makespan bound, then rebalancing). It also adds a new dealt forward kernel that reads the precomputed piece tables and remaps workgroup numbering so that load is balanced. The goal is to remove the imbalance where some workgroups receive longer ray walks than others in the few-slice forward path. In exchange the plan grows and build time increases, and the path carries many tunables (mode, beta, order) whose defaults may not suit every shape.

Result: no change. 109.6 million projections/s (median of 3 runs) (+0.3%).

```diff
diff --git a/ct_pvae_amd/_lib.py b/ct_pvae_amd/_lib.py
--- a/ct_pvae_amd/_lib.py
+++ b/ct_pvae_amd/_lib.py
@@ -76,6 +76,9 @@
                                               _vp]),
     "ctpvae_rotate_fwd_planned_f32": (_c_int, [_vp, _c_int, _c_int, _c_int, _c_int, _c_int, _c_int, _vp, _vp, _vp]),
     "ctpvae_rotate_fwd_planned_form": (_c_int, [_c_int, _c_int, _c_int, _c_int, _c_int, _c_int, _c_int]),
+    "ctpvae_rotate_fwd_plan_deal": (_c_int, [_vp, _c_int, _c_int, _c_int, _c_int, _c_int, _c_int, _vp, _vp, _vp, _vp, _vp]),
+    "ctpvae_fwd_deal_host": (_c_int, [_vp, _c_int, _vp, _c_int, _c_int, _c_int, _vp, _vp, _vp]),
+    "ctpvae_fwd_few_numbering": (_c_int, [_c_int, _c_int, _c_int, _vp, _vp]),
     "ctpvae_rotate_fwd_planned_loglik_f32": (_c_int, [_vp, _c_int, _c_int, _c_int, _c_int, _c_int, _c_int, _vp, _vp, _vp, _vp,
                                                       _c_float, _vp, _vp, _vp, _vp]),
     "ctpvae_rotate_bwd_planned_f32": (_c_int, [_vp, _c_int, _c_int, _c_int, _c_int, _c_int, _c_int, _vp, _vp, _vp]),
diff --git a/ct_pvae_amd/csrc/common.h b/ct_pvae_amd/csrc/common.h
--- a/ct_pvae_amd/csrc/common.h
+++ b/ct_pvae_amd/csrc/common.h
@@ -90,7 +90,7 @@
 enum Knob {
     kKnobNoPlan, kKnobForceGeneric, kKnobNs, kKnobG, kKnobWaves, kKnobBns, kKnobBw, kKnobSegNs, kKnobSegChunk,
     kKnobSegPpt, kKnobTiledNs, kKnobTiledG, kKnobSiddonNs, kKnobSiddonThreads, kKnobSiddonPpb, kKnobMaxSlices,
-    kKnobSiddonBwdNs, kKnobSiddonBwdChunks, kKnobNoCompact, kKnobSkew0, kKnobTiledSort, kKnobTiledPair, kKnobAffine, kKnobFakeStaticLds, kKnobFoldSums, kKnobTiledXcd, kKnobTiledWaves, kKnobTiledTh, kKnobReduceWaves, kKnobStepNs, kKnobStepLdsKb, kKnobTiledForce, kKnobBsort, kKnobMixG, kKnobMixG2, kKnobMixU1, kKnobNoMagic, kKnobMixG1, kKnobMixG3, kKnobMixU2, kKnobBrsplit, kKnobFwdFew, kKnobWtStores, kKnobBwdTail, kKnobCount
+    kKnobSiddonBwdNs, kKnobSiddonBwdChunks, kKnobNoCompact, kKnobSkew0, kKnobTiledSort, kKnobTiledPair, kKnobAffine, kKnobFakeStaticLds, kKnobFoldSums, kKnobTiledXcd, kKnobTiledWaves, kKnobTiledTh, kKnobReduceWaves, kKnobStepNs, kKnobStepLdsKb, kKnobTiledForce, kKnobBsort, kKnobMixG, kKnobMixG2, kKnobMixU1, kKnobNoMagic, kKnobMixG1, kKnobMixG3, kKnobMixU2, kKnobBrsplit, kKnobFwdFew, kKnobWtStores, kKnobBwdTail, kKnobFwdDeal, kKnobFwdDealBeta, kKnobCount
 };
 int knob(Knob k);
 
diff --git a/ct_pvae_amd/csrc/core.hip b/ct_pvae_amd/csrc/core.hip
--- a/ct_pvae_amd/csrc/core.hip
+++ b/ct_pvae_amd/csrc/core.hip
@@ -22,7 +22,7 @@
 
 static const char *const kKnobNames[kKnobCount] = {
     "NO_PLAN", "FORCE_GENERIC", "NS", "G", "WAVES", "BNS", "BW", "SEG_NS", "SEG_CHUNK", "SEG_PPT", "TILED_NS", "TILED_G",
-    "SIDDON_NS", "SIDDON_THREADS", "SIDDON_PPB", "MAX_SLICES", "SIDDON_BWD_NS", "SIDDON_BWD_CHUNKS", "NO_COMPACT", "SKEW0", "TILED_SORT", "TILED_PAIR", "AFFINE", "FAKE_STATIC_LDS", "FOLD_SUMS", "TILED_XCD", "TILED_WAVES", "TILED_TH", "REDUCE_WAVES", "STEP_NS", "STEP_LDS_KB", "TILED_FORCE", "BSORT", "MIXG", "MIXG_G2", "MIXG_U1", "NO_MAGIC", "MIXG_G1", "MIXG_G3", "MIXG_U2", "BRSPLIT", "FWD_FEW", "WT_STORES", "BWD_TAIL"};
+    "SIDDON_NS", "SIDDON_THREADS", "SIDDON_PPB", "MAX_SLICES", "SIDDON_BWD_NS", "SIDDON_BWD_CHUNKS", "NO_COMPACT", "SKEW0", "TILED_SORT", "TILED_PAIR", "AFFINE", "FAKE_STATIC_LDS", "FOLD_SUMS", "TILED_XCD", "TILED_WAVES", "TILED_TH", "REDUCE_WAVES", "STEP_NS", "STEP_LDS_KB", "TILED_FORCE", "BSORT", "MIXG", "MIXG_G2", "MIXG_U1", "NO_MAGIC", "MIXG_G1", "MIXG_G3", "MIXG_U2", "BRSPLIT", "FWD_FEW", "WT_STORES", "BWD_TAIL", "FWD_DEAL", "FWD_DEAL_BETA"};
 static std::atomic<int> g_knobs[kKnobCount];
 static int find_knob(const char *name)
 {
diff --git a/ct_pvae_amd/csrc/fwd_deal.h b/ct_pvae_amd/csrc/fwd_deal.h
--- /dev/null
+++ b/ct_pvae_amd/csrc/fwd_deal.h
@@ -0,0 +1,153 @@
+#pragma once
+#include <hip/hip_runtime.h>
+
+#include "common.h"
+
+namespace ctpvae {
+
+constexpr int kDealMaxG = 12;
+constexpr int kDealMaxTasks = 2048;
+constexpr int kFewMaxTasks = 48;
+constexpr int kDealWaves = 16;
+constexpr int kDealAlpha = 720, kDealBeta = 73;
+
+__host__ __device__ inline long long deal_piece_cost(int longest, int count, int beta = kDealBeta)
+{
+    if (count <= 0) return 0;
+    const int w = count < kDealWaves ? count : kDealWaves, rounds = (count + kDealWaves - 1) / kDealWaves;
+    return (long long)(kDealAlpha + beta * w) * longest * rounds;
+}
+__host__ __device__ inline int deal_rank(const int *len, int n, int i)
+{
+    int r = 0;
+    for (int k = 0; k < n; ++k) r += (len[k] > len[i] || (len[k] == len[i] && k < i)) ? 1 : 0;
+    return r;
+}
+__host__ __device__ inline int deal_fill(const int *slen, int n, int G, long long B, int C, int *sz, int beta)
+{
+    int s = 0;
+    for (int i = 0; i < G; ++i) {
+        int k = 0;
+        while (s + k < n && k < C && deal_piece_cost(slen[s], k + 1, beta) <= B) ++k;
+        sz[i] = k;
+        s += k;
+    }
+    return n - s;
+}
+__host__ __device__ inline void deal_sizes(const int *slen, int n, int G, int cap, int *sz, int beta = kDealBeta)
+{
+    for (int i = 0; i < G; ++i) sz[i] = 0;
+    if (n <= 0) return;
+    const int need = (n + G - 1) / G;
+    if (cap < need) cap = need;
+    long long lo = 0, hi = deal_piece_cost(slen[0], cap, beta);
+    while (lo < hi) {
+        const long long mid = lo + (hi - lo) / 2;
+        if (deal_fill(slen, n, G, mid, cap, sz, beta) == 0) hi = mid;
+        else lo = mid + 1;
+    }
+    const long long B = lo;
+    int clo = need, chi = cap;
+    while (clo < chi) {
+        const int mid = (clo + chi) / 2;
+        if (deal_fill(slen, n, G, B, mid, sz, beta) == 0) chi = mid;
+        else clo = mid + 1;
+    }
+    deal_fill(slen, n, G, B, clo, sz, beta);
+    for (;;) {
+        int r = 0;
+        for (int i = 1; i < G; ++i)
+            if (sz[i] <= sz[r]) r = i;
+        int d = -1;
+        for (int i = 0; i < G; ++i)
+            if (sz[i] >= sz[r] + 2 && (d < 0 || sz[i] > sz[d] || (sz[i] == sz[d] && (i > r ? i - r : r - i) < (d > r ? d - r : r - d)))) d = i;
+        if (d < 0) return;
+        --sz[d], ++sz[r];
+        bool ok = true;
+        for (int i = 0, s = 0; i < G; s += sz[i], ++i)
+            if (sz[i] > 0 && deal_piece_cost(slen[s], sz[i], beta) > B) ok = false;
+        if (!ok) {
+            ++sz[d], --sz[r];
+            return;
+        }
+    }
+}
+__host__ __device__ inline int deal0_count(int n, int G, int gi) { return gi < n ? (n - gi + G - 1) / G : 0; }
+__host__ __device__ inline int deal0_first(int n, int G, int gi) { return gi * (n / G) + (gi < n % G ? gi : n % G); }
+__host__ __device__ inline int deal_snake_piece(int G, int r) { const int j = r / G, k = r - j * G; return (j & 1) ? G - 1 - k : k; }
+__host__ __device__ inline int deal_snake_count(int n, int G, int gi)
+{
+    const int q = n / G, rem = n - q * G;
+    return q + (((q & 1) ? gi >= G - rem : gi < rem) ? 1 : 0);
+}
+__host__ __device__ inline int deal_snake_first(int n, int G, int gi)
+{
+    int f = 0;
+    for (int g2 = 0; g2 < gi; ++g2) f += deal_snake_count(n, G, g2);
+    return f;
+}
+__host__ __device__ inline int deal_kind_rank(const long long *cost, int nk, int kind, int mode)
+{
+    if (mode == 0) return kind;
+    int r = 0;
+    for (int k = 0; k < nk; ++k) r += (cost[k] > cost[kind] || (cost[k] == cost[kind] && k < kind)) ? 1 : 0;
+    return r;
+}
+__host__ __device__ inline int deal_wave_pos(int w, int n1, int r)
+{
+    const int f = n1 >> 2, s = w & 3, lvl = w >> 2;
+    return s >= r ? lvl * (4 - r) + (s - r) : (4 - r) * f + lvl * r + s;
+}
+
+struct FewNumbering {
+    unsigned p0, qwhole, D, inv_D, swap, noct8, wgs, inv_wgs;
+};
+__host__ __device__ inline unsigned deal_magic(unsigned d) { return d > 1 ? (unsigned)((1ull << 32) / d) + 1u : 0u; }
+__host__ __device__ inline unsigned deal_div(unsigned x, unsigned magic) { return magic ? (unsigned)(((unsigned long long)x * magic) >> 32) : x; }
+__host__ __device__ inline void few_piece_of(unsigned q, const FewNumbering &n, int &u, int &rank)
+{
+    const unsigned qw = q - n.p0;
+    if (qw < n.qwhole) {
+        const unsigned x = qw >> 3, d = deal_div(x, n.inv_D), r = x - d * n.D;
+        u = (int)((n.swap ? r : d) * 8 + (q & 7));
+        rank = (int)(n.swap ? d : r);
+    } else {
+        const unsigned rem = q < n.p0 ? q : q - n.qwhole, ru = deal_div(rem, n.inv_wgs);
+        u = (int)(n.noct8 + ru);
+        rank = (int)(rem - ru * n.wgs);
+    }
+}
+__host__ __device__ inline FewNumbering few_numbering(int units, int wgs, int mode)
+{
+    FewNumbering n;
+    const unsigned noct = (unsigned)units / 8, part = (unsigned)units - 8 * noct;
+    n.wgs = (unsigned)wgs, n.inv_wgs = deal_magic(n.wgs);
+    n.noct8 = 8 * noct, n.qwhole = 8 * noct * n.wgs;
+    n.swap = mode != 0 && noct > 0 ? 1 : 0;
+    n.D = n.swap ? noct : n.wgs, n.inv_D = deal_magic(n.D);
+    n.p0 = mode == 1 ? part * n.wgs : 0;
+    return n;
+}
+
+__host__ __device__ inline long long deal_section_words(int T) { return 4 * kDealMaxG + T; }
+inline int fwd_deal_mode() { const int v = knob(kKnobFwdDeal); return v == 0 || (v >= 2 && v <= 5) ? v : 1; }
+inline int fwd_deal_beta() { const int v = knob(kKnobFwdDealBeta); return v >= 0 ? v : kDealBeta; }
+inline int fwd_deal_table(int v) { return v == 3 || v == 4 ? 1 : (v == 5 ? 2 : 0); }
+inline int fwd_deal_order(int v) { return v == 0 || v == 4 ? 0 : (v == 2 ? 2 : 1); }
+struct DealPlanView {
+    long long off_clist, off_rng, off_deal;
+    int nJB;
+};
+struct FwdDealtArgs {
+    const uint2 *pieces, *recs;
+    const uint4 *idx;
+    int rows, cs, src_stride, pitch, zero, PW, A;
+    int st, ast;
+    int S, slice, snake;
+    FewNumbering num;
+};
+int fwd_deal_build(char *plan, int A, const DealPlanView &v, ctpvae_stream_t stream);
+int fwd_dealt_launch(int ns, unsigned grid, int waves, size_t shmem, const float *img_dev, float *sino_dev, const FwdDealtArgs &k,
+                     ctpvae_stream_t stream);
+
+}
diff --git a/ct_pvae_amd/csrc/fwd_walk.h b/ct_pvae_amd/csrc/fwd_walk.h
--- /dev/null
+++ b/ct_pvae_amd/csrc/fwd_walk.h
@@ -0,0 +1,79 @@
+#ifndef CTPVAE_FWD_WALK_H
+#define CTPVAE_FWD_WALK_H
+__device__ __forceinline__ void unpack2(unsigned pk, int &lo4, int &hi4)
+{
+    asm("v_lshlrev_b32_sdwa %0, 2, %1 dst_sel:DWORD dst_unused:UNUSED_PAD src0_sel:DWORD src1_sel:WORD_0"
+        : "=v"(lo4)
+        : "v"(pk));
+    asm("v_lshlrev_b32_sdwa %0, 2, %1 dst_sel:DWORD dst_unused:UNUSED_PAD src0_sel:DWORD src1_sel:WORD_1"
+        : "=v"(hi4)
+        : "v"(pk));
+}
+__device__ __forceinline__ float lds_at(const float *, int byte_off) { return *(lds_cptr)(size_t)(unsigned)byte_off; }
+__device__ __forceinline__ void unpack2x8(unsigned pk, int &lo8, int &hi8)
+{
+    asm("v_lshlrev_b32_sdwa %0, 3, %1 dst_sel:DWORD dst_unused:UNUSED_PAD src0_sel:DWORD src1_sel:WORD_0"
+        : "=v"(lo8)
+        : "v"(pk));
+    asm("v_lshlrev_b32_sdwa %0, 3, %1 dst_sel:DWORD dst_unused:UNUSED_PAD src0_sel:DWORD src1_sel:WORD_1"
+        : "=v"(hi8)
+        : "v"(pk));
+}
+__device__ __forceinline__ void gather8(const float *lds, const uint4 q, f32x2 (&v)[8])
+{
+    int a[8];
+    unpack2x8(q.x, a[0], a[1]);
+    unpack2x8(q.y, a[2], a[3]);
+    unpack2x8(q.z, a[4], a[5]);
+    unpack2x8(q.w, a[6], a[7]);
+#pragma unroll
+    for (int e = 0; e < 8; ++e) v[e] = *(const __attribute__((address_space(3))) f32x2 *)(size_t)(unsigned)a[e];
+}
+__device__ __forceinline__ void gather8(const float *lds, const uint4 q, float (&v)[8])
+{
+    int a0, a1, a2, a3, a4, a5, a6, a7;
+    unpack2(q.x, a0, a1);
+    unpack2(q.y, a2, a3);
+    unpack2(q.z, a4, a5);
+    unpack2(q.w, a6, a7);
+    v[0] = lds_at(lds, a0);
+    v[1] = lds_at(lds, a1);
+    v[2] = lds_at(lds, a2);
+    v[3] = lds_at(lds, a3);
+    v[4] = lds_at(lds, a4);
+    v[5] = lds_at(lds, a5);
+    v[6] = lds_at(lds, a6);
+    v[7] = lds_at(lds, a7);
+}
+
+#endif
+#define CTPVAE_PADD(VC) _Pragma("unroll") for (int e = 0; e < 8; ++e) acc += VC[e];
+#define CTPVAE_PSTEP(QN, VN, VC, LOADNEXT)    \
+                gather8(lds, QN, VN);                                                              \
+                LOADNEXT;                                                                          \
+                __builtin_amdgcn_sched_barrier(0);                                                 \
+                CTPVAE_PADD(VC)
+#define CTPVAE_FWD_WALK_U16                                                                        \
+            int n = 0;                                                                             \
+            for (; n + 4 < ng; n += 4) {    \
+                CTPVAE_PSTEP(q1, vb, va, q1 = p[st])                             \
+                CTPVAE_PSTEP(q2, va, vb, q2 = p[2 * st])                          \
+                CTPVAE_PSTEP(q3, vb, va, q3 = p[3 * st])                          \
+                CTPVAE_PSTEP(q0, va, vb, (p += 4 * st, q0 = p[0]))                \
+            }                                                                                      \
+            if (n + 1 >= ng) {    \
+                CTPVAE_PADD(va)                                                                    \
+            } else {                                                                               \
+                CTPVAE_PSTEP(q1, vb, va, (void)0)                                                  \
+                if (n + 2 >= ng) {                                                                 \
+                    CTPVAE_PADD(vb)                                                                \
+                } else {                                                                           \
+                    CTPVAE_PSTEP(q2, va, vb, (void)0)                                              \
+                    if (n + 3 >= ng) {                                                             \
+                        CTPVAE_PADD(va)                                                            \
+                    } else {                                                                       \
+                        CTPVAE_PSTEP(q3, vb, va, (void)0)                                          \
+                        CTPVAE_PADD(vb)                                                            \
+                    }                                                                              \
+                }                                                                                  \
+            }
diff --git a/ct_pvae_amd/csrc/rotate_deal.hip b/ct_pvae_amd/csrc/rotate_deal.hip
--- /dev/null
+++ b/ct_pvae_amd/csrc/rotate_deal.hip
@@ -0,0 +1,265 @@
+#include <algorithm>
+#include <atomic>
+
+#include "common.h"
+#include "fwd_deal.h"
+#include "lds_stage.h"
+#include "rotate_plan.h"
+#include "tune_stamps.h"
+
+namespace ctpvae {
+
+#include "fwd_walk.h"
+
+__global__ __launch_bounds__(1024) void rotate_fwd_deal_kernel(int A, DealPlanView L, char *__restrict__ plan, int mode, int order, int beta)
+{
+    __shared__ int len[kDealMaxTasks], slen[kDealMaxTasks], sm[kDealMaxTasks];
+    __shared__ uint2 rec[kDealMaxTasks];
+    __shared__ int sizes[kDealMaxG][2][kDealMaxG];
+    __shared__ long long cost[kDealMaxG][2 * kDealMaxG];
+    const int *clist = reinterpret_cast<const int *>(plan + L.off_clist);
+    const int *rng = reinterpret_cast<const int *>(plan + L.off_rng);
+    uint2 *table = reinterpret_cast<uint2 *>(plan + L.off_deal);
+    const int n0 = clist[0] * L.nJB, n1 = clist[A + 1] * L.nJB, T = n0 + n1;
+    const int tid = threadIdx.x;
+    for (int t = tid; t < T; t += blockDim.x) {
+        const int c = t < n0 ? 0 : 1, i = t - c * n0, ncls = clist[c * (A + 1)];
+        const int jb = i / ncls, a = clist[c * (A + 1) + 1 + (i - jb * ncls)];
+        const int first = rng[(a * L.nJB + jb) * 2], last = kRngBias - rng[(a * L.nJB + jb) * 2 + 1];
+        const int ng = last >= first ? last - first + 1 : 0, g0 = last >= first ? first : 0;
+        len[t] = ng;
+        rec[t] = make_uint2((unsigned)a | ((unsigned)jb << 16), (unsigned)g0 | ((unsigned)ng << 16));
+    }
+    __syncthreads();
+    for (int t = tid; t < T; t += blockDim.x) {
+        const int c = t < n0 ? 0 : 1, base = c * n0, i = t - base;
+        const int r = deal_rank(len + base, c ? n1 : n0, i);
+        slen[base + r] = len[t];
+        sm[base + r] = i;
+    }
+    __syncthreads();
+    if (tid < 2 * kDealMaxG) {
+        const int G = tid / 2 + 1, c = tid & 1, base = c * n0, n = c ? n1 : n0;
+        int *sz = sizes[G - 1][c];
+        if (mode == 0) {
+            for (int gi = 0; gi < G; ++gi) sz[gi] = deal0_count(n, G, gi);
+        } else if (mode == 2) {
+            for (int gi = 0; gi < G; ++gi) sz[gi] = deal_snake_count(n, G, gi);
+        } else {
+            deal_sizes(slen + base, n, G, kFewMaxTasks, sz, beta);
+        }
+        for (int gi = 0, s = 0; gi < G; s += sz[gi], ++gi) {
+            int longest = 0;
+            if (mode == 0) {
+                for (int j = 0; j < sz[gi]; ++j) longest = max(longest, len[base + j * G + gi]);
+            } else if (sz[gi] > 0) {
+                longest = slen[base + (mode == 2 ? gi : s)];
+            }
+            cost[G - 1][2 * gi + c] = deal_piece_cost(longest, sz[gi], beta);
+        }
+    }
+    __syncthreads();
+    if (tid < 2 * kDealMaxG * kDealMaxG) {
+        const int G = tid / (2 * kDealMaxG) + 1, kind = tid % (2 * kDealMaxG);
+        if (kind < 2 * G) {
+            const int c = kind & 1, gi = kind >> 1;
+            int first = c * n0;
+            for (int g2 = 0; g2 < gi; ++g2) first += sizes[G - 1][c][g2];
+            const uint2 e = make_uint2((unsigned)first, (unsigned)sizes[G - 1][c][gi] | ((unsigned)c << 31));
+            table[(size_t)(G - 1) * deal_section_words(T) + kind] = e;
+            table[(size_t)(G - 1) * deal_section_words(T) + 2 * kDealMaxG + deal_kind_rank(cost[G - 1], 2 * G, kind, order)] = e;
+        }
+    }
+    for (int x = tid; x < kDealMaxG * T; x += blockDim.x) {
+        const int G = x / T + 1, t = x - (G - 1) * T;
+        const int c = t < n0 ? 0 : 1, base = c * n0, i = t - base, n = c ? n1 : n0;
+        uint2 *recs = table + (size_t)(G - 1) * deal_section_words(T) + 4 * kDealMaxG;
+        if (mode == 0) recs[base + deal0_first(n, G, i % G) + i / G] = rec[t];
+        else if (mode == 2) recs[base + deal_snake_first(n, G, deal_snake_piece(G, i)) + i / G] = rec[base + sm[t]];
+        else recs[t] = rec[base + sm[t]];
+    }
+}
+
+template <int NS>
+__global__ __launch_bounds__(1024) void rotate_fwd_planned_kernel_dealt(const float *__restrict__ img, float *__restrict__ sino, FwdDealtArgs k)
+{
+    typedef typename SliceVec<NS>::type vec_t;
+    extern __shared__ float lds[];
+    int u, rank;
+    few_piece_of(blockIdx.x, k.num, u, rank);
+    const uint2 piece = k.pieces[rank];
+    const int c = (int)(piece.y >> 31), ntask = (int)(piece.y & 0x7fffffffu);
+    const uint2 *recs = k.recs + piece.x;
+    const int s = u * NS;
+    const bool has2 = NS == 2 && s + 1 < k.S;
+    const int lane = threadIdx.x & 63, nwaves = blockDim.x >> 6;
+    const int wave = __builtin_amdgcn_readfirstlane(threadIdx.x >> 6);
+    const float *im = img + (size_t)s * k.slice;
+    CTPVAE_PSTAMP(0);
+
+#ifdef CTPVAE_TUNE_NOIDX
+    const size_t st = 0;
+#else
+    const size_t st = (size_t)k.st;
+#endif
+    struct Task {
+        bool valid;
+        int a, j, ng;
+        const uint4 *p;
+        uint4 q0, q1, q2, q3;
+    };
+    auto fill = [&](Task &t, int pos) {
+        const uint2 r = recs[pos];
+        const int jb = (int)(r.x >> 16), g0 = (int)(r.y & 0xffffu);
+        t.a = (int)(r.x & 0xffffu);
+        t.ng = (int)(r.y >> 16);
+        t.j = lane_to_bin(k.PW, jb, lane);
+        t.p = k.idx + ((size_t)t.a * k.ast + (size_t)g0 * k.st + jb * 64) + lane;
+        t.q0 = t.p[0];
+        t.q1 = t.p[st];
+        t.q2 = t.p[2 * st];
+        t.q3 = t.p[3 * st];
+        t.p += 4 * st;
+    };
+    Task cur;
+    const int n1 = min(ntask, nwaves);
+    cur.valid = wave < n1;
+    if (cur.valid) fill(cur, deal_wave_pos(wave, n1, n1 & k.snake));
+    int *next_task = reinterpret_cast<int *>(lds + (k.zero + 1) * NS);
+    if (threadIdx.x == 0) *next_task = nwaves;
+
+    {
+        const float *srcs[NS];
+        srcs[0] = im;
+        if constexpr (NS == 2) srcs[1] = im + (has2 ? (size_t)k.slice : 0);
+        if (c == 0) stage_unit_pow2_m<NS, 8 / NS, true>(lds, srcs, k.rows, k.cs, k.src_stride, k.pitch, lane, wave, nwaves, [] {});
+        else stage_unit_pow2_m<NS, 8 / NS, false>(lds, srcs, k.rows, k.cs, k.src_stride, k.pitch, lane, wave, nwaves, [] {});
+    }
+    if (threadIdx.x < NS) lds[k.zero * NS + threadIdx.x] = 0.0f;
+    CTPVAE_PSTAMP(1);
+    __syncthreads();
+    CTPVAE_PSTAMP(2);
+
+    while (cur.valid) {
+        int m = 0;
+        if (lane == 0) m = atomicAdd(next_task, 1);
+        Task nxt;
+        {
+            const int pos = __builtin_amdgcn_readfirstlane(m);
+            nxt.valid = pos < ntask;
+            if (nxt.valid) fill(nxt, pos);
+        }
+        const int ng = __builtin_amdgcn_readfirstlane(cur.ng);
+        const uint4 *p = cur.p;
+        vec_t acc = 0.0f;
+        if (ng > 0) {
+            uint4 q0 = cur.q0, q1 = cur.q1, q2 = cur.q2, q3 = cur.q3;
+            vec_t va[8], vb[8];
+            gather8(lds, q0, va);
+            q0 = p[0];
+            CTPVAE_FWD_WALK_U16
+        }
+        if ((unsigned)cur.j < (unsigned)k.PW) {
+            const size_t o = ((size_t)s * k.A + cur.a) * k.PW + cur.j;
+            if constexpr (NS == 1) {
+                sino[o] = acc;
+            } else {
+                sino[o] = acc.x;
+                if (has2) sino[o + (size_t)k.A * k.PW] = acc.y;
+            }
+        }
+        cur = nxt;
+    }
+    CTPVAE_PSTAMP(3);
+}
+#undef CTPVAE_FWD_WALK_U16
+#undef CTPVAE_PSTEP
+#undef CTPVAE_PADD
+
+int fwd_deal_build(char *plan, int A, const DealPlanView &v, ctpvae_stream_t stream)
+{
+    const int deal = fwd_deal_mode();
+    hipLaunchKernelGGL(rotate_fwd_deal_kernel, dim3(1), dim3(1024), 0, (hipStream_t)stream, A, v, plan, fwd_deal_table(deal), fwd_deal_order(deal),
+                       fwd_deal_beta());
+    CTPVAE_LAUNCH_CHECK("rotate_fwd_deal_kernel");
+    return CTPVAE_OK;
+}
+
+int fwd_dealt_launch(int ns, unsigned grid, int waves, size_t shmem, const float *img_dev, float *sino_dev, const FwdDealtArgs &k,
+                     ctpvae_stream_t stream)
+{
+    auto launch = [&](auto kernel) -> int {
+        static std::atomic<unsigned long long> attr_set{0}, abs_ok{0};
+        CTPVAE_REQUIRE_NO_STATIC_LDS(kernel, "rotate_fwd_planned_kernel_dealt", abs_ok);
+        CTPVAE_SET_MAX_LDS_ONCE(kernel, attr_set);
+        hipLaunchKernelGGL(kernel, dim3(grid), dim3(64 * waves), shmem, (hipStream_t)stream, img_dev, sino_dev, k);
+        CTPVAE_LAUNCH_CHECK("rotate_fwd_planned_kernel_dealt");
+        return CTPVAE_OK;
+    };
+    return ns == 2 ? launch(rotate_fwd_planned_kernel_dealt<2>) : launch(rotate_fwd_planned_kernel_dealt<1>);
+}
+
+}
+
+using namespace ctpvae;
+
+extern "C" {
+
+int ctpvae_fwd_deal_host(const int *len0, int n0, const int *len1, int n1, int G, int mode, int *pieces, int *tasks, long long *cost)
+{
+    CTPVAE_REQUIRE(G >= 1 && G <= kDealMaxG && n0 >= 0 && n1 >= 0 && n0 + n1 <= kDealMaxTasks, "fwd_deal_host: 1 <= G <= %d, at most %d tasks",
+                   kDealMaxG, kDealMaxTasks);
+    CTPVAE_REQUIRE((len0 || n0 == 0) && (len1 || n1 == 0) && pieces && tasks && cost, "fwd_deal_host: null pointer");
+    const int table = fwd_deal_table(mode), order = fwd_deal_order(mode);
+    static thread_local int slen[kDealMaxTasks], sm[kDealMaxTasks];
+    int sizes[2][kDealMaxG];
+    long long kcost[2 * kDealMaxG];
+    for (int c = 0; c < 2; ++c) {
+        const int *len = c ? len1 : len0;
+        const int n = c ? n1 : n0, base = c * n0;
+        for (int i = 0; i < n; ++i) {
+            const int r = deal_rank(len, n, i);
+            slen[base + r] = len[i];
+            sm[base + r] = i;
+        }
+        if (table == 0) {
+            for (int gi = 0; gi < G; ++gi) sizes[c][gi] = deal0_count(n, G, gi);
+        } else if (table == 2) {
+            for (int gi = 0; gi < G; ++gi) sizes[c][gi] = deal_snake_count(n, G, gi);
+        } else {
+            deal_sizes(slen + base, n, G, kFewMaxTasks, sizes[c], fwd_deal_beta());
+        }
+        for (int gi = 0, s = 0; gi < G; s += sizes[c][gi], ++gi) {
+            int longest = 0;
+            if (table == 0) {
+                for (int j = 0; j < sizes[c][gi]; ++j) longest = std::max(longest, len[j * G + gi]);
+            } else if (sizes[c][gi] > 0) {
+                longest = slen[base + (table == 2 ? gi : s)];
+            }
+            kcost[2 * gi + c] = deal_piece_cost(longest, sizes[c][gi], fwd_deal_beta());
+        }
+        for (int i = 0; i < n; ++i) {
+            if (table == 0) tasks[base + deal0_first(n, G, i % G) + i / G] = i;
+            else if (table == 2) tasks[base + deal_snake_first(n, G, deal_snake_piece(G, i)) + i / G] = sm[base + i];
+            else tasks[base + i] = sm[base + i];
+        }
+    }
+    for (int kind = 0; kind < 2 * G; ++kind) {
+        const int c = kind & 1, gi = kind >> 1, r = deal_kind_rank(kcost, 2 * G, kind, order);
+        int first = c * n0;
+        for (int g2 = 0; g2 < gi; ++g2) first += sizes[c][g2];
+        pieces[4 * r + 0] = c, pieces[4 * r + 1] = gi, pieces[4 * r + 2] = first, pieces[4 * r + 3] = sizes[c][gi];
+        cost[r] = kcost[kind];
+    }
+    return CTPVAE_OK;
+}
+
+int ctpvae_fwd_few_numbering(int units, int wgs, int mode, int *unit_out, int *rank_out)
+{
+    CTPVAE_REQUIRE(units >= 1 && wgs >= 1 && (long long)units * wgs < (1ll << 28) && unit_out && rank_out, "fwd_few_numbering: bad arguments");
+    const FewNumbering n = few_numbering(units, wgs, mode);
+    for (int q = 0; q < units * wgs; ++q) few_piece_of((unsigned)q, n, unit_out[q], rank_out[q]);
+    return CTPVAE_OK;
+}
+
+}
diff --git a/ct_pvae_amd/csrc/rotate_plan.h b/ct_pvae_amd/csrc/rotate_plan.h
--- a/ct_pvae_amd/csrc/rotate_plan.h
+++ b/ct_pvae_amd/csrc/rotate_plan.h
@@ -17,6 +17,8 @@
     return lane < 32 ? c - 32 * (jb + 1) + lane : c + 32 * jb + (lane - 32);
 }
 __host__ __device__ inline int num_bin_blocks(int PW) { return (PW - (PW >> 1) + 31) / 32; }
+
+constexpr int kRngBias = 0x7f7f7f7f;
 
 typedef const __attribute__((address_space(3))) float *lds_cptr;
 typedef __attribute__((address_space(3))) float *lds_ptr;
diff --git a/ct_pvae_amd/csrc/rotate_plan.hip b/ct_pvae_amd/csrc/rotate_plan.hip
--- a/ct_pvae_amd/csrc/rotate_plan.hip
+++ b/ct_pvae_amd/csrc/rotate_plan.hip
@@ -3,8 +3,10 @@
 #include <climits>
 #include <cstdlib>
 #include <type_traits>
+#include <vector>
 
 #include "common.h"
+#include "fwd_deal.h"
 #include "lds_stage.h"
 #include "loglik_math.h"
 #include "rotate_plan.h"
@@ -58,6 +60,12 @@
     L.bytes = (long long)L.NA16 * g.H * L.Wpad * 16;
     L.bytes = (L.bytes + 255) / 256 * 256 + (long long)bwd_tail_dwords(g.A, dup) * g.H * L.Wpad * 4;
     return L;
+}
+static inline long long fwd_deal_off(const FwdLayout &L) { return (L.bytes + 255) / 256 * 256; }
+static inline long long fwd_deal_bytes(const PlanGeom &g, const FwdLayout &L)
+{
+    const long long T = (long long)g.A * L.nJB;
+    return T <= kDealMaxTasks ? kDealMaxG * deal_section_words((int)T) * 8 : 0;
 }
 static bool fwd_plan_fits(const PlanGeom &g)
 {
@@ -123,7 +131,6 @@
     }
     first[(size_t)a * L.PWpad + jb * 64 + lane] = f;
 }
-constexpr int kRngBias = 0x7f7f7f7f;
 __global__ __launch_bounds__(64) void rotate_fwd_plan_kernel(PlanGeom g, const float *__restrict__ T8, FwdLayout L,
                                                              char *__restrict__ plan)
 {
@@ -224,51 +231,7 @@
     cell[1] = (unsigned char)hit1;
 }
 
-__device__ __forceinline__ void unpack2(unsigned pk, int &lo4, int &hi4)
-{
-    asm("v_lshlrev_b32_sdwa %0, 2, %1 dst_sel:DWORD dst_unused:UNUSED_PAD src0_sel:DWORD src1_sel:WORD_0"
-        : "=v"(lo4)
-        : "v"(pk));
-    asm("v_lshlrev_b32_sdwa %0, 2, %1 dst_sel:DWORD dst_unused:UNUSED_PAD src0_sel:DWORD src1_sel:WORD_1"
-        : "=v"(hi4)
-        : "v"(pk));
-}
-__device__ __forceinline__ float lds_at(const float *, int byte_off) { return *(lds_cptr)(size_t)(unsigned)byte_off; }
-__device__ __forceinline__ void unpack2x8(unsigned pk, int &lo8, int &hi8)
-{
-    asm("v_lshlrev_b32_sdwa %0, 3, %1 dst_sel:DWORD dst_unused:UNUSED_PAD src0_sel:DWORD src1_sel:WORD_0"
-        : "=v"(lo8)
-        : "v"(pk));
-    asm("v_lshlrev_b32_sdwa %0, 3, %1 dst_sel:DWORD dst_unused:UNUSED_PAD src0_sel:DWORD src1_sel:WORD_1"
-        : "=v"(hi8)
-        : "v"(pk));
-}
-__device__ __forceinline__ void gather8(const float *lds, const uint4 q, f32x2 (&v)[8])
-{
-    int a[8];
-    unpack2x8(q.x, a[0], a[1]);
-    unpack2x8(q.y, a[2], a[3]);
-    unpack2x8(q.z, a[4], a[5]);
-    unpack2x8(q.w, a[6], a[7]);
-#pragma unroll
-    for (int e = 0; e < 8; ++e) v[e] = *(const __attribute__((address_space(3))) f32x2 *)(size_t)(unsigned)a[e];
-}
-__device__ __forceinline__ void gather8(const float *lds, const uint4 q, float (&v)[8])
-{
-    int a0, a1, a2, a3, a4, a5, a6, a7;
-    unpack2(q.x, a0, a1);
-    unpack2(q.y, a2, a3);
-    unpack2(q.z, a4, a5);
-    unpack2(q.w, a6, a7);
-    v[0] = lds_at(lds, a0);
-    v[1] = lds_at(lds, a1);
-    v[2] = lds_at(lds, a2);
-    v[3] = lds_at(lds, a3);
-    v[4] = lds_at(lds, a4);
-    v[5] = lds_at(lds, a5);
-    v[6] = lds_at(lds, a6);
-    v[7] = lds_at(lds, a7);
-}
+#include "fwd_walk.h"
 
 __host__ __device__ inline unsigned div_magic(unsigned d) { return d > 1 ? (unsigned)((1ull << 32) / d) + 1u : 0u; }
 __host__ __device__ inline unsigned div_by_magic(unsigned x, unsigned magic) { return magic ? (unsigned)(((unsigned long long)x * magic) >> 32) : x; }
@@ -301,36 +264,6 @@
 }
 
 constexpr int kSelRounds = 4;
-#define CTPVAE_PADD(VC) _Pragma("unroll") for (int e = 0; e < 8; ++e) acc += VC[e];
-#define CTPVAE_PSTEP(QN, VN, VC, LOADNEXT)    \
-                gather8(lds, QN, VN);                                                              \
-                LOADNEXT;                                                                          \
-                __builtin_amdgcn_sched_barrier(0);                                                 \
-                CTPVAE_PADD(VC)
-#define CTPVAE_FWD_WALK_U16                                                                        \
-            int n = 0;                                                                             \
-            for (; n + 4 < ng; n += 4) {    \
-                CTPVAE_PSTEP(q1, vb, va, q1 = p[st])                             \
-                CTPVAE_PSTEP(q2, va, vb, q2 = p[2 * st])                          \
-                CTPVAE_PSTEP(q3, vb, va, q3 = p[3 * st])                          \
-                CTPVAE_PSTEP(q0, va, vb, (p += 4 * st, q0 = p[0]))                \
-            }                                                                                      \
-            if (n + 1 >= ng) {    \
-                CTPVAE_PADD(va)                                                                    \
-            } else {                                                                               \
-                CTPVAE_PSTEP(q1, vb, va, (void)0)                                                  \
-                if (n + 2 >= ng) {                                                                 \
-                    CTPVAE_PADD(vb)                                                                \
-                } else {                                                                           \
-                    CTPVAE_PSTEP(q2, va, vb, (void)0)                                              \
-                    if (n + 3 >= ng) {                                                             \
-                        CTPVAE_PADD(va)                                                            \
-                    } else {                                                                       \
-                        CTPVAE_PSTEP(q3, vb, va, (void)0)                                          \
-                        CTPVAE_PADD(vb)                                                            \
-                    }                                                                              \
-                }                                                                                  \
-            }
 template <int NS, bool EPI, bool SEL>
 __global__ __launch_bounds__(1024) void rotate_fwd_planned_kernel(const float *__restrict__ img, PlanGeom g, FwdLayout L,
                                                                   const char *__restrict__ plan, int wgs_per_slice,
@@ -855,7 +788,11 @@
 {
     if (H <= 0 || W <= 0 || PH < H || PW < W || A <= 0) return fail(CTPVAE_EINVAL, "rotate_plan_bytes: bad sizes");
     const PlanGeom g{H, W, PH, PW, 0, 0, A};
-    return which == 0 ? fwd_layout(g).bytes : bwd_layout(g).bytes;
+    if (which == 0) {
+        const FwdLayout L = fwd_layout(g);
+        return fwd_deal_off(L) + fwd_deal_bytes(g, L);
+    }
+    return bwd_layout(g).bytes;
 }
 
 int ctpvae_rotate_plan_build_f32(const float *T8_dev, const float *Tinv8_dev, int A, int H, int W, int PH, int PW, int py,
@@ -879,6 +816,8 @@
         CTPVAE_LAUNCH_CHECK("rotate_fwd_plan_kernel");
         hipLaunchKernelGGL(rotate_class_list_kernel, dim3(1), dim3(64), 0, (hipStream_t)stream, A, L, (char *)fwd_plan_dev);
         CTPVAE_LAUNCH_CHECK("rotate_class_list_kernel");
+        if (fwd_deal_bytes(g, L) > 0)
+            if (int rc = fwd_deal_build((char *)fwd_plan_dev, A, DealPlanView{L.off_clist, L.off_rng, fwd_deal_off(L), L.nJB}, stream)) return rc;
     }
     if (bwd_plan_dev) {
         CTPVAE_REQUIRE(Tinv8_dev, "rotate_plan_build: backward plan needs the inverted transforms");
@@ -1088,7 +1027,6 @@
     return CTPVAE_OK;
 }
 
-constexpr int kFewMaxTasks = 48;
 static bool fwd_few_ok(const FwdShape &sh, bool dense, bool img_aligned16)
 {
     if (knob(kKnobFwdFew) == 0) return false;
@@ -1111,6 +1049,21 @@
     const int ns = sh.ns;
     if (fwd_few_ok(sh, !sel_dev && !epi.lp, (reinterpret_cast<uintptr_t>(img_dev) & 15) == 0)) {
         const char *plan = (const char *)fwd_plan_dev;
+        const int deal = fwd_deal_mode(), G = sh.wgs_per_slice / 2;
+        if (deal != 0 && G <= kDealMaxG && fwd_deal_bytes(g, L) > 0) {
+            FwdDealtArgs k;
+            const int order = sh.units >= 8 && sh.grid <= 256 && (sh.grid / 8 + 1) * (long long)(sh.units / 8 + 1) < (1ll << 32) ? fwd_deal_order(deal) : 0;
+            const uint2 *sec = reinterpret_cast<const uint2 *>(plan + fwd_deal_off(L)) + (size_t)(G - 1) * deal_section_words(A * L.nJB);
+            k.pieces = sec + (order ? 2 * kDealMaxG : 0);
+            k.recs = sec + 4 * kDealMaxG;
+            k.idx = reinterpret_cast<const uint4 *>(plan + L.off_idx);
+            k.A = A, k.rows = H, k.cs = W == 64 ? 0 : (W == 128 ? 1 : 2), k.src_stride = W, k.pitch = L.pitch, k.zero = L.zero;
+            k.PW = PW, k.st = L.PWpad, k.ast = L.Galloc * L.PWpad;
+            k.S = S, k.slice = H * W;
+            k.snake = fwd_deal_table(deal) == 0 ? 0 : 3;
+            k.num = few_numbering(sh.units, sh.wgs_per_slice, order);
+            return fwd_dealt_launch(ns, (unsigned)sh.grid, sh.waves, sh.shmem, img_dev, sino_dev, k, stream);
+        }
         FwdFewArgs k;
         k.clist = reinterpret_cast<const int *>(plan + L.off_clist);
         k.inv_ncls = reinterpret_cast<const unsigned *>(plan + L.off_clist + 2ll * (A + 1) * 4);
@@ -1153,6 +1106,33 @@
     FwdShape sh;
     if (int rc = fwd_planned_shape(S, H, W, PH, PW, A, false, 0, sh)) return rc;
     return fwd_few_ok(sh, true, img_aligned16 != 0) ? 1 : 0;
+}
+
+int ctpvae_rotate_fwd_plan_deal(const void *fwd_plan_dev, int H, int W, int PH, int PW, int A, int G, int *pieces, int *recs, int *cls,
+                                int *rng, ctpvae_stream_t stream)
+{
+    if (int rc = check_plan_geom("rotate_fwd_plan_deal", H, W, PH, PW, 0, 0, A)) return rc;
+    CTPVAE_REQUIRE(fwd_plan_dev && pieces && recs && cls && rng, "rotate_fwd_plan_deal: null pointer");
+    const PlanGeom g{H, W, PH, PW, 0, 0, A};
+    const FwdLayout L = fwd_layout(g);
+    CTPVAE_REQUIRE(G >= 1 && G <= kDealMaxG && fwd_deal_bytes(g, L) > 0, "rotate_fwd_plan_deal: the plan holds no deal for G=%d", G);
+    const int T = A * L.nJB;
+    std::vector<uint2> sec((size_t)deal_section_words(T));
+    std::vector<int> raw((size_t)T * 2);
+    const char *plan = (const char *)fwd_plan_dev;
+    CTPVAE_HIP(hipMemcpyAsync(sec.data(), plan + fwd_deal_off(L) + (size_t)(G - 1) * sec.size() * 8, sec.size() * 8, hipMemcpyDeviceToHost, (hipStream_t)stream));
+    CTPVAE_HIP(hipMemcpyAsync(raw.data(), plan + L.off_rng, raw.size() * 4, hipMemcpyDeviceToHost, (hipStream_t)stream));
+    CTPVAE_HIP(hipMemcpyAsync(cls, plan + L.off_cls, (size_t)A * 4, hipMemcpyDeviceToHost, (hipStream_t)stream));
+    CTPVAE_HIP(hipStreamSynchronize((hipStream_t)stream));
+    for (int r = 0; r < 2 * G; ++r)
+        pieces[3 * r + 0] = (int)(sec[2 * kDealMaxG + r].y >> 31), pieces[3 * r + 1] = (int)sec[2 * kDealMaxG + r].x, pieces[3 * r + 2] = (int)(sec[2 * kDealMaxG + r].y & 0x7fffffffu);
+    for (int t = 0; t < T; ++t) {
+        const uint2 v = sec[4 * kDealMaxG + t];
+        recs[4 * t + 0] = (int)(v.x & 0xffffu), recs[4 * t + 1] = (int)(v.x >> 16), recs[4 * t + 2] = (int)(v.y & 0xffffu), recs[4 * t + 3] = (int)(v.y >> 16);
+        const int first = raw[2 * t], last = kRngBias - raw[2 * t + 1];
+        rng[2 * t + 0] = last >= first ? first : 0, rng[2 * t + 1] = last >= first ? last - first + 1 : 0;
+    }
+    return CTPVAE_OK;
 }
 
 int ctpvae_rotate_fwd_planned_f32(const float *img_dev, int S, int H, int W, int PH, int PW, int A, const void *fwd_plan_dev,
diff --git a/ct_pvae_amd/forward_functions.py b/ct_pvae_amd/forward_functions.py
--- a/ct_pvae_amd/forward_functions.py
+++ b/ct_pvae_amd/forward_functions.py
@@ -316,6 +316,23 @@
         aligned = 1 if img is None or img.data_ptr() % 16 == 0 else 0
         return _lib.check(self._lib.ctpvae_rotate_fwd_planned_form(S, self.H, self.W, self.PH, self.PW, self.A, aligned),
                           "rotate_fwd_planned_form")
+
+    def forward_deal(self, G):
+        import numpy as np
+        plan = self._u16_plan if self._compact else self._fwd_plan
+        if plan is None or self.interp != _lib.NEAREST:
+            return None
+        njb = (self.PW - self.PW // 2 + 31) // 32
+        T = self.A * njb
+        if T > 2048:
+            return None
+        pieces, recs = np.zeros((2 * G, 3), np.int32), np.zeros((T, 4), np.int32)
+        cls, rng = np.zeros(self.A, np.int32), np.zeros((self.A, njb, 2), np.int32)
+        with torch.cuda.device(self.device):
+            _lib.check(self._lib.ctpvae_rotate_fwd_plan_deal(plan.data_ptr(), self.H, self.W, self.PH, self.PW, self.A, G,
+                                                             pieces.ctypes.data, recs.ctypes.data, cls.ctypes.data, rng.ctypes.data,
+                                                             _stream_ptr()), "rotate_fwd_plan_deal")
+        return {"pieces": pieces, "recs": recs, "cls": cls, "rng": rng}
 
     def _run_compact(self, img_ptr, S, out_ptr, angles_i=None, n=0, mask=None, meas=None, dense=0, pnm=None, eps=0.0,
                      lp_ptr=None, dlp_ptr=None, part_ptr=None, sum_ptr=None, noise=0):
diff --git a/include/ctpvae_radon.h b/include/ctpvae_radon.h
--- a/include/ctpvae_radon.h
+++ b/include/ctpvae_radon.h
@@ -88,6 +88,11 @@
 int ctpvae_rotate_fwd_planned_f32(const float *img_dev, int S, int H, int W, int PH, int PW, int A,
                                   const void *fwd_plan_dev, float *sino_dev, ctpvae_stream_t stream);
 int ctpvae_rotate_fwd_planned_form(int S, int H, int W, int PH, int PW, int A, int img_aligned16);
+int ctpvae_rotate_fwd_plan_deal(const void *fwd_plan_dev, int H, int W, int PH, int PW, int A, int G, int *pieces, int *recs,
+                                int *cls, int *rng, ctpvae_stream_t stream);
+int ctpvae_fwd_deal_host(const int *len0, int n0, const int *len1, int n1, int G, int mode, int *pieces, int *tasks,
+                         long long *cost);
+int ctpvae_fwd_few_numbering(int units, int wgs, int mode, int *unit_out, int *rank_out);
 int ctpvae_rotate_fwd_planned_loglik_f32(const float *img_dev, int S, int H, int W, int PH, int PW, int A,
                                          const void *fwd_plan_dev, const float *mask_dev, const float *meas_dev,
                                          const float *pnm_dev, float eps, float *sino_dev, float *lp_dev,
```
